# CityU-AIM-Group/SCAN

Hardware: AMD Instinct MI355X
Metric: train images/sec (whole node), VGG16 C2F 1024x2048 (higher is better)
Workload: dtype f32 (fp32 storage, fp32 multiply, fp32 accumulate -- the reference's arithmetic; the convolutions run it on the bf16 matrix cores as bf16x6: every fp32 operand cut into 3 bf16 pieces = all 24 significand bits, 6 bf16 MFMAs per product)

## Files before the change

include/scan_hip.h:

```cpp
#ifndef SCAN_HIP_H
#define SCAN_HIP_H

#include <stdint.h>

#ifdef __cplusplus
extern "C" {
#endif

#define SCAN_MAX_LEVELS 5

typedef struct {
  int32_t n_levels;
  int32_t n_images;
  int32_t h[SCAN_MAX_LEVELS];
  int32_t w[SCAN_MAX_LEVELS];
  int64_t row_off[SCAN_MAX_LEVELS + 1];
} scan_pyramid_t;

const char* scan_last_error(void);
int scan_abi_version(void);

#define SCAN_TUNE_UNKNOWN (-2147483647 - 1)
int scan_tune(const char* key, int value);
int scan_tune_get(const char* key);
// ... 47 lines not shown
int scan_cka_bce_forward_ordered(const float* logits, const float* act, int64_t M, int32_t Cf, float target, float* out,
                                 float* ws, void* stream);
int scan_cka_bce_forward_loss_ordered(const float* logits, const float* act, int64_t M, int32_t Cf, float target,
                                      float* out, float* ws, void* stream);
int64_t scan_softmax_focal_ordered_ws_floats(int64_t M);
int scan_softmax_focal_forward_ordered(const float* logits, const int64_t* labels, int64_t M, int32_t K, float gamma,
                                       float* loss_sum, float* ws, void* stream);

int scan_scale(const float* x, float alpha, float* y, int64_t n, void* stream);
int scan_copy_cols(const float* src, int32_t ld_src, float* dst, int32_t ld_dst, int64_t M, int32_t ncols, int32_t ztail,
                   void* stream);
int scan_paradigm_update(float* P, const float* pb, int32_t K, int32_t C, int32_t T, int32_t it, void* stream);

int32_t scan_dynconv_max_classes(void);
int scan_dynconv_softmax_forward(const float* feat, const float* kernels, int64_t M, int32_t C, int32_t K,
                                 float* logits, float* probs, void* stream);
int64_t scan_dynconv_ws_floats(int64_t M, int32_t C, int32_t K);
int scan_dynconv_softmax_backward(const float* feat, const float* kernels, const float* probs,
                                  const float* d_logits_in, const float* d_probs, int64_t M, int32_t C,
                                  int32_t K, float* d_feat, float* d_kernels, float* ws, void* stream);

int scan_softmax_focal_forward(const float* logits, const int64_t* labels, int64_t M, int32_t K, float gamma,
                               float* loss_sum, void* stream);
int scan_softmax_focal_backward(const float* logits, const int64_t* labels, int64_t M, int32_t K, float gamma,
                                float d_scale, float* d_logits, void* stream);

#define SCAN_NMS_PANEL 8192
#define SCAN_NMS_MAX 262144
int64_t scan_nms_ws_bytes(int64_t n);
int scan_nms(const float* dets, const float* scores, const float* labels, int64_t n, float thr, int32_t rule_ge,
             int64_t* keep_out, int32_t* num_keep_out, void* workspace, void* stream);

int scan_conv2d_forward(const float* x, const scan_pyramid_t* xd, int32_t Cin_s, const float* w, const float* bias,
                        float* y, const scan_pyramid_t* yd, int32_t Cout, int32_t Cout_s, int32_t ksize,
                        int32_t stride, int32_t relu, void* stream);
int scan_conv2d_dgrad(const float* dy, const scan_pyramid_t* yd, int32_t Cout_s, const float* wt, float* dx,
                      const scan_pyramid_t* xd, int32_t Cin, int32_t Cin_s, int32_t ksize, int32_t stride,
                      const float* mask, void* stream);
int64_t scan_conv2d_wgrad_ws_floats(const scan_pyramid_t* yd, int32_t Cin_s, int32_t Cout, int32_t ksize);
int scan_conv2d_wgrad(const float* x, const scan_pyramid_t* xd, int32_t Cin_s, const float* dy,
                      const scan_pyramid_t* yd, int32_t Cout, int32_t Cout_s, int32_t ksize, int32_t stride,
                      float* dw, int32_t accumulate, float* ws, void* stream);
int scan_weight_split(const float* w, int32_t O, int32_t T, int32_t Cs, int32_t mode, void* wh, void* wl,
                      int32_t Csw, void* stream);
int scan_conv3x3_bf16x3(const float* x, const scan_pyramid_t* d, int32_t Cs, const void* wh, const void* wl,
                        int32_t Csw, const float* bias, const float* mask, float* y, int32_t Nout, int32_t Ns,
                        int32_t relu, void* stream);
int scan_conv1x1_bf16x3(const float* x, const scan_pyramid_t* xd, int32_t Cs, const void* wh, const void* wl,
                        int32_t Csw, const float* bias, const float* mask, float* y, const scan_pyramid_t* yd,
                        int32_t Nout, int32_t Ns, int32_t relu, int32_t map, void* stream);
int64_t scan_conv1x1_wgrad_bf16x3_ws_floats(const scan_pyramid_t* yd, int32_t Cs, int32_t Cout);
int scan_conv1x1_wgrad_bf16x3(const float* x, const scan_pyramid_t* xd, int32_t Cs, const float* dy,
                              const scan_pyramid_t* yd, int32_t Cout, int32_t Cout_s, int32_t stride, float* dw,
                              float* db, int32_t accumulate, float* ws, void* stream);
int scan_conv_smallcin_bf16x3(const float* x, int32_t N, int32_t H, int32_t W, const float* w, const float* bias,
                              float* y, int32_t Cout, int32_t Cout_s, int32_t ksize, int32_t stride, int32_t relu,
                              void* stream);
int scan_conv3x3_gn_bf16x3(const float* x, const scan_pyramid_t* d, int32_t Cs, const void* wh, const void* wl,
                           int32_t Csw, const float* bias, float* y, int32_t Nout, int32_t Ns, float* gn_ws,
                           void* stream);
int scan_conv3x3_gn_acc_bf16x3(const float* x, const scan_pyramid_t* d, int32_t Cs, const void* wh, const void* wl,
                               int32_t Csw, const float* bias, float* y, int32_t Nout, int32_t Ns, float* gn_ws,
                               void* stream);
int scan_groupnorm_stats_from_sums(const float* ws, const scan_pyramid_t* d, int32_t C, int32_t G, float eps,
                                   float* stats, void* stream);
int scan_conv3x3_pool2_bf16x3(const float* x, const scan_pyramid_t* d, int32_t Cs, const void* wh, const void* wl,
                              int32_t Csw, const float* bias, float* y, int32_t Nout, int32_t Ns, int32_t relu,
                              void* stream);
int64_t scan_conv3x3_wgrad_bf16x3_ws_floats(const scan_pyramid_t* d, int32_t Cs, int32_t Cout);
int scan_conv3x3_wgrad_bf16x3(const float* x, const scan_pyramid_t* d, int32_t Cs, const float* dy, int32_t Cout,
                              int32_t Cout_s, float* dw, float* db, int32_t accumulate, float* ws, void* stream);
int scan_weight_split3(const float* w, int32_t O, int32_t T, int32_t Cs, int32_t mode, void* wh, void* wm, void* wl,
                       int32_t Csw, void* stream);
int scan_conv3x3_bf16x6(const float* x, const scan_pyramid_t* d, int32_t Cs, const void* wh, const void* wm,
                        const void* wl, int32_t Csw, const float* bias, const float* mask, float* y, int32_t Nout,
                        int32_t Ns, int32_t relu, void* stream);
int scan_conv1x1_bf16x6(const float* x, const scan_pyramid_t* xd, int32_t Cs, const void* wh, const void* wm,
                        const void* wl, int32_t Csw, const float* bias, const float* mask, float* y,
                        const scan_pyramid_t* yd, int32_t Nout, int32_t Ns, int32_t relu, int32_t map, void* stream);
int scan_conv3x3_gn_bf16x6(const float* x, const scan_pyramid_t* d, int32_t Cs, const void* wh, const void* wm,
                           const void* wl, int32_t Csw, const float* bias, float* y, int32_t Nout, int32_t Ns,
                           float* gn_ws, int32_t clear, void* stream);
int scan_conv3x3_pool2_bf16x6(const float* x, const scan_pyramid_t* d, int32_t Cs, const void* wh, const void* wm,
                              const void* wl, int32_t Csw, const float* bias, float* y, int32_t Nout, int32_t Ns,
                              int32_t relu, void* stream);
int scan_conv_smallcin_bf16x6(const float* x, int32_t N, int32_t H, int32_t W, const float* w, const float* bias,
                              float* y, int32_t Cout, int32_t Cout_s, int32_t ksize, int32_t stride, int32_t relu,
                              void* stream);
int64_t scan_conv3x3_wgrad_bf16x6_ws_floats(const scan_pyramid_t* d, int32_t Cs, int32_t Cout);
int scan_conv3x3_wgrad_bf16x6(const float* x, const scan_pyramid_t* d, int32_t Cs, const float* dy, int32_t Cout,
                              int32_t Cout_s, float* dw, float* db, int32_t accumulate, float* ws, void* stream);
int64_t scan_conv1x1_wgrad_bf16x6_ws_floats(const scan_pyramid_t* yd, int32_t Cs, int32_t Cout);
int scan_conv1x1_wgrad_bf16x6(const float* x, const scan_pyramid_t* xd, int32_t Cs, const float* dy,
                              const scan_pyramid_t* yd, int32_t Cout, int32_t Cout_s, int32_t stride, float* dw,
                              float* db, int32_t accumulate, float* ws, void* stream);
int scan_conv3x3_bf16x6_instance(const scan_pyramid_t* d, int32_t Nout);
int scan_conv3x3_wino_bf16x6(const float* x, const scan_pyramid_t* d, int32_t Cs, const void* wh, const void* wm,
                             const void* wl, int32_t Csw, const float* bias, const float* mask, float* y, int32_t Nout,
                             int32_t Ns, int32_t relu, float* gn_ws, int32_t clear, void* stream);
int scan_conv3x3_bf16x6_wino(int32_t Nout, int32_t Csw);
#define SCAN_CONV_SUMS 1
#define SCAN_CONV_POOL 2
#define SCAN_CONV_DIRECT3X3 0
#define SCAN_CONV_WINO3X3 1
#define SCAN_CONV_1X1 2
typedef struct {
  int32_t pieces;
  int32_t taps;
  int32_t dgrad;
  int32_t O, Cs_w;
  int32_t split_mode;
  int32_t plane_rows;
  int32_t plane_taps;
  int32_t csw;
  int32_t nout;
  int32_t rem;
  int32_t family;
  int32_t instance;
  int32_t flags;
} scan_conv_plan_t;
int scan_conv_plan(int32_t pieces, int32_t taps, int32_t dgrad, int32_t O, int32_t Cs_w, int32_t Cs_src,
                   const scan_pyramid_t* od, int32_t flags, scan_conv_plan_t* plan);
int scan_conv_weight_split(const scan_conv_plan_t* plan, const float* w, void* p0, void* p1, void* p2, void* stream);
int scan_conv_run(const scan_conv_plan_t* plan, const float* x, const scan_pyramid_t* xd, int32_t Cs, const void* p0,
                  const void* p1, const void* p2, const float* bias, const float* mask, float* y,
                  const scan_pyramid_t* yd, int32_t Ns, int32_t relu, int32_t map, float* gn_ws, int32_t clear,
                  void* stream);
#define SCAN_WGRAD_SPLIT3X3 1
#define SCAN_WGRAD_SPLIT1X1 2
#define SCAN_WGRAD_GENERIC 3
#define SCAN_WGRAD_FP32 0
#define SCAN_WGRAD_V4 1
#define SCAN_WGRAD_V6_64X32 2
#define SCAN_WGRAD_V6_32X64 3
#define SCAN_WGRAD_V6_32X64_WINO 4
typedef struct {
  int32_t family;
  int32_t pieces;
  int32_t ksize;
  int32_t stride;
  int32_t Cs, Cout;
  int32_t variant;
  int32_t wk;
  int32_t n_tiles;
  int32_t c_tiles;
  int32_t splits;
  int32_t cps;
  int32_t slab_taps;
  int32_t fused_db;
  int64_t chunks;
  int64_t slab_floats;
  int64_t bias_off;
  int64_t colsum_off;
  int64_t ws_floats;
} scan_conv_wgrad_plan_t;
int scan_conv_wgrad_plan(int32_t pieces, int32_t ksize, int32_t stride, int32_t Cs, int32_t Cout, const scan_pyramid_t* xd,
                         const scan_pyramid_t* yd, scan_conv_wgrad_plan_t* plan);
int scan_conv_wgrad_run(const scan_conv_wgrad_plan_t* plan, const float* x, const scan_pyramid_t* xd, int32_t Cs,
                        const float* dy, const scan_pyramid_t* yd, int32_t Cout, int32_t Cout_s, float* dw, float* db,
                        int32_t accumulate, float* ws, void* stream);
int scan_weight_transpose(const float* w, int32_t Cout, int32_t T, int32_t Cin_s, float* wt, int32_t Cout_s,
                          void* stream);
int64_t scan_colsum_ws_floats(int64_t M, int32_t C);
int scan_colsum(const float* dy, int64_t M, int32_t C, int32_t ld, float* db, int32_t accumulate, float* ws,
                void* stream);
int scan_relu_backward(const float* dy, const float* y, float* out, int64_t n, void* stream);

int scan_groupnorm_stats(const float* x, const scan_pyramid_t* d, int32_t C, int32_t G, float eps, float* stats,
                         float* ws, void* stream);
int scan_groupnorm_relu_forward(const float* x, const scan_pyramid_t* d, int32_t C, int32_t G, const float* stats,
                                const float* gamma, const float* beta, int32_t relu, float* y, void* stream);
int scan_groupnorm_relu_forward_from_sums(const float* x, const scan_pyramid_t* d, int32_t C, int32_t G,
                                          const float* sums, float eps, const float* gamma, const float* beta,
                                          int32_t relu, float* y, float* stats, void* stream);
int64_t scan_groupnorm_ws_floats(const scan_pyramid_t* d, int32_t C, int32_t G);
int scan_groupnorm_relu_backward(const float* x, const float* beta, const float* dy, const scan_pyramid_t* d, int32_t C,
                                 int32_t G, const float* stats, const float* gamma, int32_t relu, float* dx,
                                 float* dgamma, float* dbeta, int32_t accumulate, float* ws, void* stream);
int scan_groupnorm_relu_forward_ld(const float* x, const scan_pyramid_t* d, int32_t C, int32_t G, const float* stats,
                                   const float* gamma, const float* beta, int32_t relu, float* y, int32_t ldy,
                                   void* stream);
int scan_groupnorm_relu_forward_from_sums_ld(const float* x, const scan_pyramid_t* d, int32_t C, int32_t G,
                                             const float* sums, float eps, const float* gamma, const float* beta,
                                             int32_t relu, float* y, int32_t ldy, float* stats, void* stream);
int scan_groupnorm_relu_backward_ld(const float* x, const float* beta, const float* dy, int32_t lddy,
                                    const scan_pyramid_t* d, int32_t C, int32_t G, const float* stats, const float* gamma,
                                    int32_t relu, float* dx, float* dgamma, float* dbeta, int32_t accumulate, float* ws,
                                    void* stream);
int64_t scan_groupnorm_ordered_ws_floats(const scan_pyramid_t* d, int32_t C, int32_t G);
int scan_groupnorm_stats_ordered(const float* x, const scan_pyramid_t* d, int32_t C, int32_t G, float eps, float* stats,
                                 float* ws, void* stream);
int scan_groupnorm_relu_backward_ordered(const float* x, const float* beta, const float* dy, const scan_pyramid_t* d,
                                         int32_t C, int32_t G, const float* stats, const float* gamma, int32_t relu,
                                         float* dx, float* dgamma, float* dbeta, int32_t accumulate, float* ws,
                                         void* stream);
int scan_groupnorm_relu_backward_ld_ordered(const float* x, const float* beta, const float* dy, int32_t lddy,
                                            const scan_pyramid_t* d, int32_t C, int32_t G, const float* stats,
                                            const float* gamma, int32_t relu, float* dx, float* dgamma, float* dbeta,
                                            int32_t accumulate, float* ws, void* stream);
#define SCAN_GN_SUMS 1
#define SCAN_GN_SEPARATE_FINAL 2
#define SCAN_GN_FROM_X 0
#define SCAN_GN_FROM_SUMS 1
#define SCAN_GN_FROM_SUMS_FINAL 2
typedef struct {
  int32_t C, G;
  int32_t n_levels;
  int32_t n_images;
  int32_t blocks;
  int32_t ordered;
  int32_t source;
  int32_t stats_floats;
  int32_t fwd_ws_doubles;
  int32_t bwd_ws_doubles;
} scan_groupnorm_plan_t;
int scan_groupnorm_plan(const scan_pyramid_t* d, int32_t C, int32_t G, int32_t flags, scan_groupnorm_plan_t* plan);
int scan_groupnorm_run_forward(const scan_groupnorm_plan_t* plan, const float* x, const scan_pyramid_t* d, const float* sums,
                               float eps, const float* gamma, const float* beta, int32_t relu, float* y, int32_t ldy,
                               float* stats, float* ws, void* stream);
int scan_groupnorm_run_backward(const scan_groupnorm_plan_t* plan, const float* x, const float* beta, const float* dy,
                                int32_t lddy, const scan_pyramid_t* d, const float* stats, const float* gamma, int32_t relu,
                                float* dx, float* dgamma, float* dbeta, int32_t accumulate, float* ws, int32_t ws_cleared,
                                void* stream);

int scan_fcos_assign(const scan_pyramid_t* d, const int32_t* strides, const float* soi, const float* boxes,
                     const int64_t* glabels, const int32_t* ng, int32_t G, int64_t* labels, int32_t* labels_i32,
                     float* reg, int32_t* level_pos, void* stream);
int scan_fcos_compact(const scan_pyramid_t* d, const int64_t* labels, int32_t* pos_list, int32_t* neg_list, void* stream);
int64_t scan_fcos_nodes_count(const scan_pyramid_t* d, const int32_t* level_pos);
int scan_fcos_nodes(const scan_pyramid_t* d, const int32_t* level_pos, const int64_t* labels, const float* reg,
                    const int32_t* pos_list, const int32_t* neg_list, int64_t* node_index, int64_t* node_labels,
                    int64_t* pos_inds, float* reg_pos, float* ctr_pos, void* stream);

int64_t scan_atss_assign_ws_bytes(const scan_pyramid_t* d, int32_t G, int32_t topk);
int scan_atss_assign(const scan_pyramid_t* d, const int32_t* strides, const float* anchor_sizes, const float* boxes,
                     const int64_t* glabels, const int32_t* ng, int32_t G, int32_t topk, int64_t* labels,
                     int32_t* labels_i32, int32_t* matched, int32_t* level_pos, void* ws, void* stream);
int scan_atss_targets(const scan_pyramid_t* d, const int32_t* strides, const float* anchor_sizes, const int32_t* level_pos,
                      const float* boxes, int32_t G, const int32_t* matched, const int32_t* pos_list, int64_t* pos_inds,
                      float* reg_pos, float* ctr_pos, void* stream);
int scan_atss_giou_forward(const scan_pyramid_t* d, const int32_t* strides, const float* anchor_sizes, const float* pred,
                           const float* target, const int64_t* rows, const float* weight, int64_t P, float* out2,
                           void* stream);
int64_t scan_atss_giou_ordered_ws_floats(int64_t P);
int scan_atss_giou_forward_ordered(const scan_pyramid_t* d, const int32_t* strides, const float* anchor_sizes,
                                   const float* pred, const float* target, const int64_t* rows, const float* weight,
                                   int64_t P, float* out2, float* ws, void* stream);
int scan_atss_giou_backward(const scan_pyramid_t* d, const int32_t* strides, const float* anchor_sizes, const float* pred,
                            const float* target, const int64_t* rows, const float* weight, int64_t P,
                            const float* g_num_dev, float* d_pred, void* stream);

int scan_upsample2x_add(const float* lat, const float* coarse, int32_t N, int32_t h, int32_t w, int32_t C, float* y,
                        void* stream);
int scan_downsample2x_sum(const float* g, int32_t N, int32_t h, int32_t w, int32_t C, float* d, void* stream);

int scan_maxpool2x2_forward(const float* x, int32_t N, int32_t H, int32_t W, int32_t C, float* y, void* stream);
int scan_maxpool2x2_backward(const float* x, const float* y, const float* dy, int32_t N, int32_t H, int32_t W,
                             int32_t C, float* dx, int32_t relu_mask, void* stream);

int scan_maxpool3x3s2_forward(const float* x, int32_t N, int32_t H, int32_t W, int32_t C, float* y, void* stream);
int scan_add_relu(const float* a, const float* b, float* y, int64_t n, void* stream);

#define SCAN_DBSCAN_MAX 1200000
int64_t scan_dbscan_ws_bytes(int64_t n);
int scan_dbscan_prepare(const float* pts, int64_t n, int32_t D, float eps, int32_t min_samples, void* ws,
                        int32_t* info, void* stream);
int scan_dbscan_neighbor_counts(int64_t n, const void* ws, int32_t* counts, void* stream);
int scan_dbscan_bfs_step(int64_t n, void* ws, int32_t parity, int32_t* changed, void* stream);
int scan_dbscan_finish(int64_t n, void* ws, uint8_t* in_cluster0, void* stream);

int scan_sgd_momentum(float* p, const float* g, float* buf, int64_t n, float lr, float wd, float momentum,
                      int32_t first_step, void* stream);

#define SCAN_SGD_MAX_SEGMENTS 32
typedef struct {
  float* p;
  const float* g;
  float* buf;
  int64_t n;
  float lr;
  float wd;
  int32_t first_step;
  int32_t reserved;
} scan_sgd_segment_t;
int scan_sgd_momentum_multi(const scan_sgd_segment_t* segs, int32_t n_segs, float momentum, void* stream);

#define SCAN_SPLIT_JOB_WORDS 11
int64_t scan_weight_split_job_blocks(int32_t O, int32_t T, int32_t Cs, int32_t mode, int32_t Csw);
int scan_weight_split_batched(const int64_t* jobs, int32_t n_jobs, int32_t job_words, int64_t total_blocks, void* stream);

#define SCAN_CKA_MAX_CLASSES 16
typedef struct {
  const float* w0;
  const float* b0;
  const float* w2;
  const float* b2;
} scan_cka_branch_t;
int scan_cka_stack_weights(const scan_cka_branch_t* branches, int32_t Cf, int32_t C, int32_t H, int64_t s1o, int64_t s1c,
                           int64_t s1k, int64_t s2c, int64_t s2k, int32_t Cs1, int32_t Cs2, float* w1, float* b1,
                           float* w2, float* b2, void* stream);
int scan_cka_unstack_grads(const scan_cka_branch_t* grads, int32_t Cf, int32_t C, int32_t H, int64_t s1o, int64_t s1c,
                           int64_t s1k, int64_t s2c, int64_t s2k, int32_t Cs1, int32_t Cs2, const float* dw1,
                           const float* db1, const float* dw2, const float* db2, int32_t accumulate, void* stream);

int64_t scan_gconv3x3_to1_ws_floats(const scan_pyramid_t* d, int32_t G, int32_t Cg);
int scan_gconv3x3_to1_forward(const float* x, const scan_pyramid_t* d, int32_t G, int32_t Cg, const float* w,
                              const float* bias, float* y, int32_t Ns, float* ws, void* stream);
int scan_gconv3x3_to1_dgrad(const float* dy, int32_t Ns, const scan_pyramid_t* d, int32_t G, int32_t Cg, const float* w,
                            const float* mask, float* dx, void* stream);
int scan_gconv3x3_to1_wgrad(const float* x, const float* dy, int32_t Ns, const scan_pyramid_t* d, int32_t G, int32_t Cg,
                            float* dw, int32_t accumulate, float* ws, void* stream);
int scan_gconv3x3_to1_backward(const float* x, const float* dy, int32_t Ns, const scan_pyramid_t* d, int32_t G, int32_t Cg,
                               const float* w, int32_t relu_mask, float* dx, float* dw, int32_t accumulate, float* ws,
                               void* stream);
int32_t scan_gconv3x3_to1_max_groups(void);
int scan_gconv3x3_to1_any_forward(const float* x, const scan_pyramid_t* d, int32_t G, int32_t Cg, const float* w,
                                  const float* bias, float* y, int32_t Ns, float* ws, void* stream);
int scan_gconv3x3_to1_any_dgrad(const float* dy, int32_t Ns, const scan_pyramid_t* d, int32_t G, int32_t Cg, const float* w,
                                const float* mask, float* dx, void* stream);
int scan_gconv3x3_to1_any_wgrad(const float* x, const float* dy, int32_t Ns, const scan_pyramid_t* d, int32_t G, int32_t Cg,
                                float* dw, int32_t accumulate, float* ws, void* stream);
int scan_gconv3x3_to1_any_backward(const float* x, const float* dy, int32_t Ns, const scan_pyramid_t* d, int32_t G, int32_t Cg,
                                   const float* w, int32_t relu_mask, float* dx, float* dw, int32_t accumulate, float* ws,
                                   void* stream);
int scan_gconv3x3_to1_forward_bits(const float* x, const scan_pyramid_t* d, int32_t G, int32_t Cg, const float* w,
                                   const float* bias, float* y, int32_t Ns, float* ws, uint32_t* relu_bits, void* stream);
int scan_gconv3x3_to1_backward_bits(const float* x, const float* dy, int32_t Ns, const scan_pyramid_t* d, int32_t G,
                                    int32_t Cg, const float* w, const uint32_t* relu_bits, float* dx, float* dw,
                                    int32_t accumulate, float* ws, void* stream);

int scan_resize_bilinear_u8(const uint8_t* src, int32_t H, int32_t W, uint8_t* tmp, uint8_t* dst, int32_t OH, int32_t OW,
                            const int32_t* xbounds, const int32_t* xcoef, int32_t kx, const int32_t* ybounds,
                            const int32_t* ycoef, int32_t ky, void* stream);

int scan_normalize_image_u8(const uint8_t* src, int32_t H, int32_t W, int32_t flip, int32_t to_bgr255,
                            const float* mean3, const float* std3, float* dst, int32_t Hp, int32_t Wp, int32_t layout,
                            void* stream);

int scan_take_images_backward(const float* g, const scan_pyramid_t* d, int32_t i0, int32_t i1, int32_t C, float* out,
                              void* stream);

int scan_cond_rnn_forward(const float* x, int32_t K, int32_t T, const float* const* weights, float* h0, float* h1,
                          float* kernels, void* stream);
int64_t scan_cond_rnn_ws_floats(void);
int scan_cond_rnn_backward(const float* x, int32_t K, int32_t T, const float* const* weights, const float* h0,
                           const float* h1, const float* dkernels, float* const* grads, float* ws, void* stream);

#define SCAN_PACK_MAX_LEVELS 8
typedef struct {
  const float* data;
  int32_t h, w;
  int64_t sn, sc, sy, sx;
} scan_level_t;
int scan_pyramid_pack(const scan_level_t* levels, int32_t n_levels, int32_t n_images, int32_t C, float* rows, int32_t Cs,
                      void* stream);
int scan_pyramid_unpack(const float* rows, int32_t Cs, const scan_level_t* levels, int32_t n_levels, int32_t n_images,
                        int32_t C, void* stream);

int scan_deform_sample_forward(const float* x, const scan_pyramid_t* d, int32_t C, int32_t Cs, const float* off, int32_t ld_off,
                               const float* mask, int32_t ld_mask, float* cols, void* stream);
int scan_deform_sample_backward(const float* x, const scan_pyramid_t* d, int32_t C, int32_t Cs, const float* dcols, const float* off,
                                int32_t ld_off, const float* mask, int32_t ld_mask, float* doff, int32_t ld_doff, float* dmask,
                                int32_t ld_dmask, int32_t* keys, float* wgts, void* stream);
int scan_deform_dx_gather(const float* dcols, const int64_t* perm, const int64_t* seg_start, const float* wgts, int64_t M, int32_t C,
                          int32_t Cs, float* dx, void* stream);

int scan_center_aware_map(const float* cls, int32_t Cs, int32_t C, const float* ctr, int64_t ctr_stride, float weight, int64_t M,
                          float* atten, void* stream);
int scan_row_scale_levels(const float* x, int32_t ldx, const float* a, const float* s, const scan_pyramid_t* d, int32_t C, float* y,
                          int32_t ldy, void* stream);
int scan_row_scale_levels_ptrs(const float* const* x_levels, int32_t ldx, const float* a, const float* s, const scan_pyramid_t* d,
                               int32_t C, float* y, int32_t ldy, void* stream);

#ifdef __cplusplus
}
#endif
#endif
```

scan_amd/_lib.py:

```python
import ctypes
import os

_HERE = os.path.dirname(os.path.abspath(__file__))
LIB_PATH = os.environ.get("SCAN_HIP_LIB") or os.path.join(_HERE, "libscan_hip.so")

MAX_LEVELS = 5
TUNE_UNKNOWN = -2 ** 31
NMS_PANEL = 8192
NMS_MAX = 262144

c_i32, c_i64, c_f32, c_vp = ctypes.c_int32, ctypes.c_int64, ctypes.c_float, ctypes.c_void_p


class PyramidDesc(ctypes.Structure):
    _fields_ = [("n_levels", c_i32), ("n_images", c_i32), ("h", c_i32 * MAX_LEVELS), ("w", c_i32 * MAX_LEVELS),
                ("row_off", c_i64 * (MAX_LEVELS + 1))]


_PD = ctypes.POINTER(PyramidDesc)


class SgdSegment(ctypes.Structure):
    _fields_ = [("p", c_vp), ("g", c_vp), ("buf", c_vp), ("n", c_i64), ("lr", c_f32), ("wd", c_f32),
                ("first_step", c_i32), ("reserved", c_i32)]


class CkaBranch(ctypes.Structure):
    _fields_ = [("w0", c_vp), ("b0", c_vp), ("w2", c_vp), ("b2", c_vp)]


class LevelDesc(ctypes.Structure):
    _fields_ = [("data", c_vp), ("h", c_i32), ("w", c_i32), ("sn", c_i64), ("sc", c_i64), ("sy", c_i64), ("sx", c_i64)]


class ConvPlan(ctypes.Structure):
    _fields_ = [(n, c_i32) for n in ("pieces", "taps", "dgrad", "O", "Cs_w", "split_mode", "plane_rows", "plane_taps", "csw",
                                     "nout", "rem", "family", "instance", "flags")]


CONV_SUMS, CONV_POOL = 1, 2
_CP = ctypes.POINTER(ConvPlan)


class WgradPlan(ctypes.Structure):
    _fields_ = [(n, c_i32) for n in ("family", "pieces", "ksize", "stride", "Cs", "Cout", "variant", "wk", "n_tiles", "c_tiles",
                                     "splits", "cps", "slab_taps", "fused_db")] + \
               [(n, c_i64) for n in ("chunks", "slab_floats", "bias_off", "colsum_off", "ws_floats")]


WGRAD_SPLIT3X3, WGRAD_SPLIT1X1, WGRAD_GENERIC = 1, 2, 3
WGRAD_FP32, WGRAD_V4, WGRAD_V6_64X32, WGRAD_V6_32X64, WGRAD_V6_32X64_WINO = range(5)
_WP = ctypes.POINTER(WgradPlan)



class GroupNormPlan(ctypes.Structure):
    _fields_ = [(n, c_i32) for n in ("C", "G", "n_levels", "n_images", "blocks", "ordered", "source", "stats_floats",
                                     "fwd_ws_doubles", "bwd_ws_doubles")]


GN_SUMS, GN_SEPARATE_FINAL = 1, 2
GN_FROM_X, GN_FROM_SUMS, GN_FROM_SUMS_FINAL = range(3)
_GP = ctypes.POINTER(GroupNormPlan)

PACK_MAX_LEVELS = 8
SGD_MAX_SEGMENTS = 32
CKA_MAX_CLASSES = 16
SPLIT_JOB_WORDS = 11

SIGNATURES = {
    "scan_last_error": (ctypes.c_char_p, []),
    "scan_abi_version": (ctypes.c_int, []),
    "scan_comm_standin": (ctypes.c_int, [ctypes.c_void_p, ctypes.c_int64, ctypes.c_double, ctypes.c_int32, ctypes.c_double,
                                         ctypes.c_void_p]),
    "scan_tune": (ctypes.c_int, [ctypes.c_char_p, ctypes.c_int]),
    "scan_take_images_backward": (ctypes.c_int, [c_vp, _PD, c_i32, c_i32, c_i32, c_vp, c_vp]),
    "scan_cond_rnn_forward": (ctypes.c_int, [c_vp, c_i32, c_i32, c_vp, c_vp, c_vp, c_vp, c_vp]),
    "scan_cond_rnn_ws_floats": (ctypes.c_int64, []),
    "scan_cond_rnn_backward": (ctypes.c_int, [c_vp, c_i32, c_i32, c_vp, c_vp, c_vp, c_vp, c_vp, c_vp, c_vp]),
    "scan_tune_get": (ctypes.c_int, [ctypes.c_char_p]),
    "scan_tune_default": (ctypes.c_int, [ctypes.c_char_p]),
    "scan_tune_key": (ctypes.c_char_p, [ctypes.c_int]),
    "scan_mfma_sustained_bf16": (ctypes.c_int, [ctypes.c_double, c_i32, ctypes.POINTER(ctypes.c_double), c_vp]),
    "scan_conv3x3_bf16x3_instance": (ctypes.c_int, [_PD, c_i32]),
    "scan_conv1x1_bf16x6_instance": (ctypes.c_int, [_PD, c_i32, c_i32]),
    "scan_conv3x3_bf16x6_instance": (ctypes.c_int, [_PD, c_i32]),
    "scan_conv3x3_bf16x6_wino": (ctypes.c_int, [c_i32, c_i32]),
    "scan_conv3x3_wino_bf16x6": (ctypes.c_int, [c_vp, _PD, c_i32, c_vp, c_vp, c_vp, c_i32, c_vp, c_vp, c_vp, c_i32, c_i32, c_i32,
                                                c_vp, c_i32, c_vp]),
    "scan_conv_plan": (ctypes.c_int, [c_i32, c_i32, c_i32, c_i32, c_i32, c_i32, _PD, c_i32, _CP]),
    "scan_conv_weight_split": (ctypes.c_int, [_CP, c_vp, c_vp, c_vp, c_vp, c_vp]),
    "scan_conv_run": (ctypes.c_int, [_CP, c_vp, _PD, c_i32, c_vp, c_vp, c_vp, c_vp, c_vp, c_vp, _PD, c_i32, c_i32, c_i32, c_vp,
                                     c_i32, c_vp]),
    "scan_conv_wgrad_plan": (ctypes.c_int, [c_i32, c_i32, c_i32, c_i32, c_i32, _PD, _PD, _WP]),
    "scan_conv_wgrad_run": (ctypes.c_int, [_WP, c_vp, _PD, c_i32, c_vp, _PD, c_i32, c_i32, c_vp, c_vp, c_i32, c_vp, c_vp]),
    "scan_sigmoid_focal_loss_forward": (ctypes.c_int, [c_vp, c_vp, c_i64, c_i32, c_f32, c_f32, c_vp, c_vp, c_vp]),
    "scan_sigmoid_focal_loss_backward": (ctypes.c_int, [c_vp, c_vp, c_vp, c_f32, c_i64, c_i32, c_f32, c_f32, c_vp, c_vp]),
    "scan_iou_loss_forward": (ctypes.c_int, [c_vp, c_vp, c_vp, c_i64, c_vp, c_vp]),
    "scan_iou_loss_backward": (ctypes.c_int, [c_vp, c_vp, c_vp, c_i64, c_vp, c_vp, c_vp]),
    "scan_bce_logits_forward": (ctypes.c_int, [c_vp, c_vp, c_f32, c_vp, c_i64, c_i64, c_vp, c_vp]),
    "scan_bce_logits_backward": (ctypes.c_int, [c_vp, c_vp, c_f32, c_vp, c_i64, c_i64, c_vp, c_vp, c_vp]),
    "scan_cka_bce_forward": (ctypes.c_int, [c_vp, c_vp, c_i64, c_i32, c_f32, c_vp, c_vp]),
    "scan_cka_bce_backward": (ctypes.c_int, [c_vp, c_vp, c_i64, c_i32, c_f32, c_vp, c_vp, c_vp]),
    "scan_cka_bce_forward_loss": (ctypes.c_int, [c_vp, c_vp, c_i64, c_i32, c_f32, c_vp, c_vp]),
    "scan_cka_bce_backward_loss": (ctypes.c_int, [c_vp, c_vp, c_i64, c_i32, c_f32, c_vp, c_vp, c_vp, c_vp]),
    "scan_scale": (ctypes.c_int, [c_vp, c_f32, c_vp, c_i64, c_vp]),
    "scan_copy_cols": (ctypes.c_int, [c_vp, c_i32, c_vp, c_i32, c_i64, c_i32, c_i32, c_vp]),
    "scan_paradigm_update": (ctypes.c_int, [c_vp, c_vp, c_i32, c_i32, c_i32, c_i32, c_vp]),
    "scan_dynconv_softmax_forward": (ctypes.c_int, [c_vp, c_vp, c_i64, c_i32, c_i32, c_vp, c_vp, c_vp]),
    "scan_dynconv_ws_floats": (c_i64, [c_i64, c_i32, c_i32]),
    "scan_dynconv_max_classes": (c_i32, []),
    "scan_dynconv_softmax_backward": (ctypes.c_int, [c_vp, c_vp, c_vp, c_vp, c_vp, c_i64, c_i32, c_i32, c_vp, c_vp, c_vp, c_vp]),
    "scan_softmax_focal_forward": (ctypes.c_int, [c_vp, c_vp, c_i64, c_i32, c_f32, c_vp, c_vp]),
    "scan_softmax_focal_backward": (ctypes.c_int, [c_vp, c_vp, c_i64, c_i32, c_f32, c_f32, c_vp, c_vp]),
    "scan_nms_ws_bytes": (c_i64, [c_i64]),
    "scan_nms": (ctypes.c_int, [c_vp, c_vp, c_vp, c_i64, c_f32, c_i32, c_vp, c_vp, c_vp, c_vp]),
    "scan_conv2d_forward": (ctypes.c_int, [c_vp, _PD, c_i32, c_vp, c_vp, c_vp, _PD, c_i32, c_i32, c_i32, c_i32, c_i32, c_vp]),
    "scan_conv2d_dgrad": (ctypes.c_int, [c_vp, _PD, c_i32, c_vp, c_vp, _PD, c_i32, c_i32, c_i32, c_i32, c_vp, c_vp]),
    "scan_conv2d_wgrad_ws_floats": (c_i64, [_PD, c_i32, c_i32, c_i32]),
    "scan_conv2d_wgrad": (ctypes.c_int, [c_vp, _PD, c_i32, c_vp, _PD, c_i32, c_i32, c_i32, c_i32, c_vp, c_i32, c_vp, c_vp]),
    "scan_weight_split": (ctypes.c_int, [c_vp, c_i32, c_i32, c_i32, c_i32, c_vp, c_vp, c_i32, c_vp]),
    "scan_conv3x3_bf16x3": (ctypes.c_int, [c_vp, _PD, c_i32, c_vp, c_vp, c_i32, c_vp, c_vp, c_vp, c_i32, c_i32, c_i32, c_vp]),
    "scan_conv3x3_wgrad_bf16x3_ws_floats": (c_i64, [_PD, c_i32, c_i32]),
    "scan_dbscan_ws_bytes": (c_i64, [c_i64]),
    "scan_conv1x1_wgrad_bf16x3_ws_floats": (c_i64, [_PD, c_i32, c_i32]),
    "scan_conv3x3_wgrad_bf16x3": (ctypes.c_int, [c_vp, _PD, c_i32, c_vp, c_i32, c_i32, c_vp, c_vp, c_i32, c_vp, c_vp]),
    "scan_weight_transpose": (ctypes.c_int, [c_vp, c_i32, c_i32, c_i32, c_vp, c_i32, c_vp]),
    "scan_colsum_ws_floats": (c_i64, [c_i64, c_i32]),
    "scan_colsum": (ctypes.c_int, [c_vp, c_i64, c_i32, c_i32, c_vp, c_i32, c_vp, c_vp]),
    "scan_relu_backward": (ctypes.c_int, [c_vp, c_vp, c_vp, c_i64, c_vp]),
    "scan_groupnorm_stats": (ctypes.c_int, [c_vp, _PD, c_i32, c_i32, c_f32, c_vp, c_vp, c_vp]),
    "scan_groupnorm_relu_forward": (ctypes.c_int, [c_vp, _PD, c_i32, c_i32, c_vp, c_vp, c_vp, c_i32, c_vp, c_vp]),
    "scan_groupnorm_relu_forward_from_sums": (ctypes.c_int, [c_vp, _PD, c_i32, c_i32, c_vp, c_f32, c_vp, c_vp, c_i32, c_vp, c_vp, c_vp]),
    "scan_groupnorm_ws_floats": (c_i64, [_PD, c_i32, c_i32]),
    "scan_fcos_assign": (ctypes.c_int, [_PD, c_vp, c_vp, c_vp, c_vp, c_vp, c_i32, c_vp, c_vp, c_vp, c_vp, c_vp]),
    "scan_fcos_compact": (ctypes.c_int, [_PD, c_vp, c_vp, c_vp, c_vp]),
    "scan_fcos_nodes_count": (c_i64, [_PD, c_vp]),
    "scan_fcos_nodes": (ctypes.c_int, [_PD, c_vp, c_vp, c_vp, c_vp, c_vp, c_vp, c_vp, c_vp, c_vp, c_vp, c_vp]),
    "scan_atss_assign_ws_bytes": (c_i64, [_PD, c_i32, c_i32]),
    "scan_atss_assign": (ctypes.c_int, [_PD, c_vp, c_vp, c_vp, c_vp, c_vp, c_i32, c_i32, c_vp, c_vp, c_vp, c_vp, c_vp, c_vp]),
    "scan_atss_targets": (ctypes.c_int, [_PD, c_vp, c_vp, c_vp, c_vp, c_i32, c_vp, c_vp, c_vp, c_vp, c_vp, c_vp]),
    "scan_atss_giou_forward": (ctypes.c_int, [_PD, c_vp, c_vp, c_vp, c_vp, c_vp, c_vp, c_i64, c_vp, c_vp]),
    "scan_atss_giou_ordered_ws_floats": (c_i64, [c_i64]),
    "scan_atss_giou_forward_ordered": (ctypes.c_int, [_PD, c_vp, c_vp, c_vp, c_vp, c_vp, c_vp, c_i64, c_vp, c_vp, c_vp]),
    "scan_atss_giou_backward": (ctypes.c_int, [_PD, c_vp, c_vp, c_vp, c_vp, c_vp, c_vp, c_i64, c_vp, c_vp, c_vp]),
    "scan_groupnorm_relu_forward_ld": (ctypes.c_int, [c_vp, _PD, c_i32, c_i32, c_vp, c_vp, c_vp, c_i32, c_vp, c_i32, c_vp]),
    "scan_groupnorm_relu_forward_from_sums_ld": (ctypes.c_int, [c_vp, _PD, c_i32, c_i32, c_vp, c_f32, c_vp, c_vp, c_i32, c_vp,
                                                                c_i32, c_vp, c_vp]),
    "scan_groupnorm_relu_backward_ld": (ctypes.c_int, [c_vp, c_vp, c_vp, c_i32, _PD, c_i32, c_i32, c_vp, c_vp, c_i32, c_vp,
                                                       c_vp, c_vp, c_i32, c_vp, c_vp]),
    "scan_groupnorm_relu_backward": (ctypes.c_int, [c_vp, c_vp, c_vp, _PD, c_i32, c_i32, c_vp, c_vp, c_i32, c_vp, c_vp, c_vp, c_i32, c_vp, c_vp]),
    "scan_maxpool2x2_forward": (ctypes.c_int, [c_vp, c_i32, c_i32, c_i32, c_i32, c_vp, c_vp]),
    "scan_maxpool2x2_backward": (ctypes.c_int, [c_vp, c_vp, c_vp, c_i32, c_i32, c_i32, c_i32, c_vp, c_i32, c_vp]),
    "scan_conv3x3_gn_bf16x3": (ctypes.c_int, [c_vp, _PD, c_i32, c_vp, c_vp, c_i32, c_vp, c_vp, c_i32, c_i32, c_vp, c_vp]),
    "scan_conv3x3_gn_acc_bf16x3": (ctypes.c_int, [c_vp, _PD, c_i32, c_vp, c_vp, c_i32, c_vp, c_vp, c_i32, c_i32, c_vp, c_vp]),
    "scan_groupnorm_stats_from_sums": (ctypes.c_int, [c_vp, _PD, c_i32, c_i32, c_f32, c_vp, c_vp]),
    "scan_conv3x3_pool2_bf16x3": (ctypes.c_int, [c_vp, _PD, c_i32, c_vp, c_vp, c_i32, c_vp, c_vp, c_i32, c_i32, c_i32, c_vp]),
    "scan_conv1x1_bf16x3": (ctypes.c_int, [c_vp, _PD, c_i32, c_vp, c_vp, c_i32, c_vp, c_vp, c_vp, _PD, c_i32, c_i32, c_i32,
                                           c_i32, c_vp]),
    "scan_conv1x1_wgrad_bf16x3": (ctypes.c_int, [c_vp, _PD, c_i32, c_vp, _PD, c_i32, c_i32, c_i32, c_vp, c_vp, c_i32, c_vp,
                                                 c_vp]),
    "scan_conv_smallcin_bf16x3": (ctypes.c_int, [c_vp, c_i32, c_i32, c_i32, c_vp, c_vp, c_vp, c_i32, c_i32, c_i32, c_i32,
                                                 c_i32, c_vp]),
    "scan_weight_split3": (ctypes.c_int, [c_vp, c_i32, c_i32, c_i32, c_i32, c_vp, c_vp, c_vp, c_i32, c_vp]),
    "scan_conv3x3_bf16x6": (ctypes.c_int, [c_vp, _PD, c_i32, c_vp, c_vp, c_vp, c_i32, c_vp, c_vp, c_vp, c_i32, c_i32, c_i32, c_vp]),
    "scan_conv1x1_bf16x6": (ctypes.c_int, [c_vp, _PD, c_i32, c_vp, c_vp, c_vp, c_i32, c_vp, c_vp, c_vp, _PD, c_i32, c_i32, c_i32,
                                           c_i32, c_vp]),
    "scan_conv3x3_gn_bf16x6": (ctypes.c_int, [c_vp, _PD, c_i32, c_vp, c_vp, c_vp, c_i32, c_vp, c_vp, c_i32, c_i32, c_vp, c_i32,
                                              c_vp]),
    "scan_conv3x3_pool2_bf16x6": (ctypes.c_int, [c_vp, _PD, c_i32, c_vp, c_vp, c_vp, c_i32, c_vp, c_vp, c_i32, c_i32, c_i32,
                                                 c_vp]),
    "scan_conv3x3_wgrad_bf16x6_ws_floats": (c_i64, [_PD, c_i32, c_i32]),
    "scan_conv3x3_wgrad_bf16x6": (ctypes.c_int, [c_vp, _PD, c_i32, c_vp, c_i32, c_i32, c_vp, c_vp, c_i32, c_vp, c_vp]),
    "scan_conv1x1_wgrad_bf16x6_ws_floats": (c_i64, [_PD, c_i32, c_i32]),
    "scan_conv1x1_wgrad_bf16x6": (ctypes.c_int, [c_vp, _PD, c_i32, c_vp, _PD, c_i32, c_i32, c_i32, c_vp, c_vp, c_i32, c_vp,
                                                 c_vp]),
    "scan_conv_smallcin_bf16x6": (ctypes.c_int, [c_vp, c_i32, c_i32, c_i32, c_vp, c_vp, c_vp, c_i32, c_i32, c_i32, c_i32,
                                                 c_i32, c_vp]),
    "scan_maxpool3x3s2_forward": (ctypes.c_int, [c_vp, c_i32, c_i32, c_i32, c_i32, c_vp, c_vp]),
    "scan_upsample2x_add": (ctypes.c_int, [c_vp, c_vp, c_i32, c_i32, c_i32, c_i32, c_vp, c_vp]),
    "scan_downsample2x_sum": (ctypes.c_int, [c_vp, c_i32, c_i32, c_i32, c_i32, c_vp, c_vp]),
    "scan_add_relu": (ctypes.c_int, [c_vp, c_vp, c_vp, c_i64, c_vp]),
    "scan_dbscan_prepare": (ctypes.c_int, [c_vp, c_i64, c_i32, c_f32, c_i32, c_vp, c_vp, c_vp]),
    "scan_dbscan_neighbor_counts": (ctypes.c_int, [c_i64, c_vp, c_vp, c_vp]),
    "scan_dbscan_bfs_step": (ctypes.c_int, [c_i64, c_vp, c_i32, c_vp, c_vp]),
    "scan_dbscan_finish": (ctypes.c_int, [c_i64, c_vp, c_vp, c_vp]),
    "scan_sgd_momentum": (ctypes.c_int, [c_vp, c_vp, c_vp, c_i64, c_f32, c_f32, c_f32, c_i32, c_vp]),
    "scan_sgd_momentum_multi": (ctypes.c_int, [ctypes.POINTER(SgdSegment), c_i32, c_f32, c_vp]),
    "scan_weight_split_job_blocks": (c_i64, [c_i32, c_i32, c_i32, c_i32, c_i32]),
    "scan_weight_split_batched": (ctypes.c_int, [c_vp, c_i32, c_i32, c_i64, c_vp]),
    "scan_cka_stack_weights": (ctypes.c_int, [ctypes.POINTER(CkaBranch), c_i32, c_i32, c_i32, c_i64, c_i64, c_i64, c_i64,
                                              c_i64, c_i32, c_i32, c_vp, c_vp, c_vp, c_vp, c_vp]),
    "scan_cka_unstack_grads": (ctypes.c_int, [ctypes.POINTER(CkaBranch), c_i32, c_i32, c_i32, c_i64, c_i64, c_i64, c_i64,
                                              c_i64, c_i32, c_i32, c_vp, c_vp, c_vp, c_vp, c_i32, c_vp]),
    "scan_gconv3x3_to1_ws_floats": (c_i64, [_PD, c_i32, c_i32]),
    "scan_gconv3x3_to1_max_groups": (c_i32, []),
    "scan_gconv3x3_to1_any_forward": (ctypes.c_int, [c_vp, _PD, c_i32, c_i32, c_vp, c_vp, c_vp, c_i32, c_vp, c_vp]),
    "scan_gconv3x3_to1_any_dgrad": (ctypes.c_int, [c_vp, c_i32, _PD, c_i32, c_i32, c_vp, c_vp, c_vp, c_vp]),
    "scan_gconv3x3_to1_any_wgrad": (ctypes.c_int, [c_vp, c_vp, c_i32, _PD, c_i32, c_i32, c_vp, c_i32, c_vp, c_vp]),
    "scan_gconv3x3_to1_any_backward": (ctypes.c_int, [c_vp, c_vp, c_i32, _PD, c_i32, c_i32, c_vp, c_i32, c_vp, c_vp, c_i32,
                                                      c_vp, c_vp]),
    "scan_gconv3x3_to1_forward": (ctypes.c_int, [c_vp, _PD, c_i32, c_i32, c_vp, c_vp, c_vp, c_i32, c_vp, c_vp]),
    "scan_gconv3x3_to1_dgrad": (ctypes.c_int, [c_vp, c_i32, _PD, c_i32, c_i32, c_vp, c_vp, c_vp, c_vp]),
    "scan_gconv3x3_to1_wgrad": (ctypes.c_int, [c_vp, c_vp, c_i32, _PD, c_i32, c_i32, c_vp, c_i32, c_vp, c_vp]),
    "scan_gconv3x3_to1_backward": (ctypes.c_int, [c_vp, c_vp, c_i32, _PD, c_i32, c_i32, c_vp, c_i32, c_vp, c_vp, c_i32, c_vp,
                                                  c_vp]),
    "scan_gconv3x3_to1_forward_bits": (ctypes.c_int, [c_vp, _PD, c_i32, c_i32, c_vp, c_vp, c_vp, c_i32, c_vp, c_vp, c_vp]),
    "scan_gconv3x3_to1_backward_bits": (ctypes.c_int, [c_vp, c_vp, c_i32, _PD, c_i32, c_i32, c_vp, c_vp, c_vp, c_vp, c_i32,
                                                       c_vp, c_vp]),
    "scan_resize_bilinear_u8": (ctypes.c_int, [c_vp, c_i32, c_i32, c_vp, c_vp, c_i32, c_i32, c_vp, c_vp, c_i32, c_vp, c_vp,
                                               c_i32, c_vp]),
    "scan_sigmoid_focal_loss_ordered_ws_floats": (c_i64, [c_i64, c_i32]),
    "scan_sigmoid_focal_loss_forward_ordered": (ctypes.c_int, [c_vp, c_vp, c_i64, c_i32, c_f32, c_f32, c_vp, c_vp, c_vp, c_vp]),
    "scan_iou_loss_ordered_ws_floats": (c_i64, [c_i64]),
    "scan_iou_loss_forward_ordered": (ctypes.c_int, [c_vp, c_vp, c_vp, c_i64, c_vp, c_vp, c_vp]),
    "scan_bce_logits_ordered_ws_floats": (c_i64, [c_i64]),
    "scan_bce_logits_forward_ordered": (ctypes.c_int, [c_vp, c_vp, c_f32, c_vp, c_i64, c_i64, c_vp, c_vp, c_vp]),
    "scan_cka_bce_ordered_ws_floats": (c_i64, [c_i64, c_i32]),
    "scan_cka_bce_forward_ordered": (ctypes.c_int, [c_vp, c_vp, c_i64, c_i32, c_f32, c_vp, c_vp, c_vp]),
    "scan_cka_bce_forward_loss_ordered": (ctypes.c_int, [c_vp, c_vp, c_i64, c_i32, c_f32, c_vp, c_vp, c_vp]),
    "scan_softmax_focal_ordered_ws_floats": (c_i64, [c_i64]),
    "scan_softmax_focal_forward_ordered": (ctypes.c_int, [c_vp, c_vp, c_i64, c_i32, c_f32, c_vp, c_vp, c_vp]),
    "scan_groupnorm_ordered_ws_floats": (c_i64, [_PD, c_i32, c_i32]),
    "scan_groupnorm_stats_ordered": (ctypes.c_int, [c_vp, _PD, c_i32, c_i32, c_f32, c_vp, c_vp, c_vp]),
    "scan_groupnorm_relu_backward_ordered": (ctypes.c_int, [c_vp, c_vp, c_vp, _PD, c_i32, c_i32, c_vp, c_vp, c_i32, c_vp, c_vp, c_vp,
                                                            c_i32, c_vp, c_vp]),
    "scan_groupnorm_relu_backward_ld_ordered": (ctypes.c_int, [c_vp, c_vp, c_vp, c_i32, _PD, c_i32, c_i32, c_vp, c_vp, c_i32, c_vp,
                                                               c_vp, c_vp, c_i32, c_vp, c_vp]),
    "scan_groupnorm_plan": (ctypes.c_int, [_PD, c_i32, c_i32, c_i32, _GP]),
    "scan_groupnorm_run_forward": (ctypes.c_int, [_GP, c_vp, _PD, c_vp, c_f32, c_vp, c_vp, c_i32, c_vp, c_i32, c_vp, c_vp, c_vp]),
    "scan_groupnorm_run_backward": (ctypes.c_int, [_GP, c_vp, c_vp, c_vp, c_i32, _PD, c_vp, c_vp, c_i32, c_vp, c_vp, c_vp, c_i32,
                                                   c_vp, c_i32, c_vp]),
    "scan_normalize_image_u8": (ctypes.c_int, [c_vp, c_i32, c_i32, c_i32, c_i32, ctypes.POINTER(c_f32),
                                               ctypes.POINTER(c_f32), c_vp, c_i32, c_i32, c_i32, c_vp]),
    "scan_pyramid_pack": (ctypes.c_int, [ctypes.POINTER(LevelDesc), c_i32, c_i32, c_i32, c_vp, c_i32, c_vp]),
    "scan_pyramid_unpack": (ctypes.c_int, [c_vp, c_i32, ctypes.POINTER(LevelDesc), c_i32, c_i32, c_i32, c_vp]),
    "scan_deform_sample_forward": (ctypes.c_int, [c_vp, _PD, c_i32, c_i32, c_vp, c_i32, c_vp, c_i32, c_vp, c_vp]),
    "scan_deform_sample_backward": (ctypes.c_int, [c_vp, _PD, c_i32, c_i32, c_vp, c_vp, c_i32, c_vp, c_i32, c_vp, c_i32, c_vp,
                                                   c_i32, c_vp, c_vp, c_vp]),
    "scan_deform_dx_gather": (ctypes.c_int, [c_vp, c_vp, c_vp, c_vp, c_i64, c_i32, c_i32, c_vp, c_vp]),
    "scan_center_aware_map": (ctypes.c_int, [c_vp, c_i32, c_i32, c_vp, c_i64, c_f32, c_i64, c_vp, c_vp]),
    "scan_row_scale_levels": (ctypes.c_int, [c_vp, c_i32, c_vp, ctypes.POINTER(c_f32), _PD, c_i32, c_vp, c_i32, c_vp]),
    "scan_row_scale_levels_ptrs": (ctypes.c_int, [ctypes.POINTER(c_vp), c_i32, c_vp, ctypes.POINTER(c_f32), _PD, c_i32, c_vp, c_i32,
                                                  c_vp]),
}

_lib = None


def lib():
    global _lib
    if _lib is None:
        if not os.path.exists(LIB_PATH):
            raise RuntimeError(
                "scan_amd: %s is missing -- build it with `python -c 'import __graft_entry__ as g; g.build()'` "
                "(hipcc --offload-arch=gfx950); there is no CPU fallback." % LIB_PATH)
        import torch
        L = ctypes.CDLL(LIB_PATH)
        for name, (res, args) in SIGNATURES.items():
            fn = getattr(L, name)
            fn.restype = res
            fn.argtypes = args
        for kv in filter(None, os.environ.get("SCAN_TUNE", "").split(",")):
            key, _, val = kv.partition("=")
            if L.scan_tune(key.strip().encode(), int(val)) == TUNE_UNKNOWN:
                raise RuntimeError("SCAN_TUNE: unknown key %r" % key)
        _lib = L
    return _lib


def tune_state():
    L, out, i = lib(), {}, 0
    while True:
        k = L.scan_tune_key(i)
        if k is None:
            return out
        out[k.decode()] = (L.scan_tune_get(k), L.scan_tune_default(k))
        i += 1


def lib_identity():
    import hashlib
    with open(LIB_PATH, "rb") as f:
        sha = hashlib.sha1(f.read()).hexdigest()
    product = os.path.realpath(LIB_PATH) == os.path.realpath(os.path.join(_HERE, "libscan_hip.so"))
    return {"lib": os.path.basename(LIB_PATH), "lib_sha1": sha, "product_library": product,
            "scan_tune_non_default": {k: v for k, (v, d) in tune_state().items() if v != d}}


def call(name, *args):
    rc = getattr(lib(), name)(*args)
    if rc != 0:
        raise RuntimeError("%s failed (%d): %s" % (name, rc, lib().scan_last_error().decode()))


def query(name, *args):
    return getattr(lib(), name)(*args)
```

scan_amd/csrc/batched.hip:

```cpp
#include "conv_split.h"

#define SPLIT_ELEMS_PER_BLOCK 2048
#define SPLIT_TILE 64

__device__ __forceinline__ void split8_store(const float (&v)[8], __bf16* __restrict__ w0, __bf16* __restrict__ w1,
                                             __bf16* __restrict__ w2, int64_t i) {
  bf16x8 q0, q1, q2;
#pragma unroll
  for (int k = 0; k < 8; ++k) {
    __bf16 q[3];
    split1_np<3>(v[k], q);
    q0[k] = q[0];
    q1[k] = q[1];
    q2[k] = q[2];
  }
  *reinterpret_cast<bf16x8*>(w0 + i) = q0;
  *reinterpret_cast<bf16x8*>(w1 + i) = q1;
  if (w2 != nullptr) *reinterpret_cast<bf16x8*>(w2 + i) = q2;
}

__global__ __launch_bounds__(256) void weight_split_batched_kernel(const int64_t* __restrict__ jobs, int n_jobs) {
  __shared__ float tile[SPLIT_TILE][SPLIT_TILE + 1];
  int j = 0;
  for (int i = 1; i < n_jobs; ++i)
    if ((int64_t)blockIdx.x >= jobs[(int64_t)i * SCAN_SPLIT_JOB_WORDS + 9]) j = i;
  const int64_t* job = jobs + (int64_t)j * SCAN_SPLIT_JOB_WORDS;
  const float* __restrict__ w = reinterpret_cast<const float*>(job[0]);
  __bf16* __restrict__ wh = reinterpret_cast<__bf16*>(job[1]);
  __bf16* __restrict__ wl = reinterpret_cast<__bf16*>(job[2]);
  __bf16* __restrict__ w2 = reinterpret_cast<__bf16*>(job[10]);
  const int O = (int)job[3], T = (int)job[4], Cs = (int)job[5], mode = (int)job[6], rows = (int)job[7],
            Csw = (int)job[8];
  const int64_t blk = (int64_t)blockIdx.x - job[9];
  const int tid = threadIdx.x;
  if (mode == 2) {
    const int64_t total = (int64_t)rows * 12 * Csw;
    const int64_t i = blk * SPLIT_ELEMS_PER_BLOCK + (int64_t)tid * 8;
    if (i >= total) return;
    const int col = (int)(i % Csw);
    const int64_t rt = i / Csw;
    const int tt = (int)(rt % 12), row = (int)(rt / 12);
    const int j = tt / 3, ky = tt - 3 * j;
    const float* src = w + ((int64_t)row * T + ky * 3) * Cs + col;
    float v[8];
#pragma unroll
    for (int k = 0; k < 8; ++k) {
      const bool in = col + k < Cs;
      v[k] = wino_g(j, in ? src[k] : 0.f, in ? src[Cs + k] : 0.f, in ? src[2 * Cs + k] : 0.f);
    }
    split8_store(v, wh, wl, w2, i);
    return;
  }
  if (mode == 0) {
    const int64_t total = (int64_t)rows * T * Csw;
    const int64_t i = blk * SPLIT_ELEMS_PER_BLOCK + (int64_t)tid * 8;
    if (i >= total) return;
    const int col = (int)(i % Csw);
    const int64_t rt = i / Csw;
    const float* src = w + rt * Cs + col;
    float v[8];
    if (col + 8 <= Cs && (Cs & 3) == 0) {
      const float4 a = *reinterpret_cast<const float4*>(src);
      const float4 b = *reinterpret_cast<const float4*>(src + 4);
      v[0] = a.x; v[1] = a.y; v[2] = a.z; v[3] = a.w;
      v[4] = b.x; v[5] = b.y; v[6] = b.z; v[7] = b.w;
    } else {
#pragma unroll
      for (int k = 0; k < 8; ++k) v[k] = (col + k < Cs) ? src[k] : 0.f;
    }
    split8_store(v, wh, wl, w2, i);
    return;
  }
  const int tiles_o = (Csw + SPLIT_TILE - 1) / SPLIT_TILE, tiles_c = (rows + SPLIT_TILE - 1) / SPLIT_TILE;
  const int to = (int)(blk % tiles_o);
  const int tc = (int)((blk / tiles_o) % tiles_c);
  const int tt = (int)(blk / ((int64_t)tiles_o * tiles_c));
  const int TO = mode == 3 ? 12 : T;
  const int o0 = to * SPLIT_TILE, c0 = tc * SPLIT_TILE;
  {
    const int cl = (tid & 15) * 4, ol = tid >> 4;
#pragma unroll
    for (int p = 0; p < SPLIT_TILE / 16; ++p) {
      const int o = o0 + ol + 16 * p, c = c0 + cl;
      float4 a = make_float4(0.f, 0.f, 0.f, 0.f);
      if (o < O && c < Cs) {
        auto read4 = [&](int t) {
          const float* src = w + ((int64_t)o * T + t) * Cs + c;
          float4 r = make_float4(0.f, 0.f, 0.f, 0.f);
          if (c + 4 <= Cs && (Cs & 3) == 0) {
            r = *reinterpret_cast<const float4*>(src);
          } else {
            r.x = src[0];
            if (c + 1 < Cs) r.y = src[1];
            if (c + 2 < Cs) r.z = src[2];
            if (c + 3 < Cs) r.w = src[3];
          }
          return r;
        };
        if (mode == 1) {
          a = read4(T - 1 - tt);
        } else {
          const int j = tt / 3, ky = tt - 3 * j;
          const float4 g0 = read4(8 - ky * 3), g1 = read4(7 - ky * 3), g2 = read4(6 - ky * 3);
          a = make_float4(wino_g(j, g0.x, g1.x, g2.x), wino_g(j, g0.y, g1.y, g2.y), wino_g(j, g0.z, g1.z, g2.z),
                          wino_g(j, g0.w, g1.w, g2.w));
        }
      }
      float* t = &tile[ol + 16 * p][cl];
      t[0] = a.x; t[1] = a.y; t[2] = a.z; t[3] = a.w;
    }
  }
  __syncthreads();
  {
    const int o8 = (tid & 7) * 8, cl = tid >> 3;
#pragma unroll
    for (int p = 0; p < SPLIT_TILE / 32; ++p) {
      const int c = c0 + cl + 32 * p, o = o0 + o8;
      if (c < rows && o < Csw) {
        float v[8];
#pragma unroll
        for (int k = 0; k < 8; ++k) v[k] = tile[o8 + k][cl + 32 * p];
        split8_store(v, wh, wl, w2, ((int64_t)c * TO + tt) * Csw + o);
      }
    }
  }
}

extern "C" int64_t scan_weight_split_job_blocks(int32_t O, int32_t T, int32_t Cs, int32_t mode, int32_t Csw) {
  const int64_t TO = mode >= 2 ? 12 : T;
  if (mode == 0 || mode == 2) return ((int64_t)O * TO * Csw + SPLIT_ELEMS_PER_BLOCK - 1) / SPLIT_ELEMS_PER_BLOCK;
  const int64_t tiles_o = (Csw + SPLIT_TILE - 1) / SPLIT_TILE, tiles_c = (Cs + SPLIT_TILE - 1) / SPLIT_TILE;
  return tiles_o * tiles_c * TO;
}

extern "C" int scan_weight_split_batched(const int64_t* jobs, int32_t n_jobs, int32_t job_words, int64_t total_blocks,
                                         void* stream) {
  SCAN_CHECK_ARG(job_words == SCAN_SPLIT_JOB_WORDS, "weight_split_batched: records of %d words, this library reads %d",
                 job_words, SCAN_SPLIT_JOB_WORDS);
  SCAN_CHECK_ARG(jobs && n_jobs > 0 && total_blocks > 0 && total_blocks < (1ll << 31),
                 "weight_split_batched: bad arguments (n_jobs=%d)", n_jobs);
  hipLaunchKernelGGL(weight_split_batched_kernel, dim3((unsigned)total_blocks), dim3(256), 0, as_stream(stream), jobs,
                     n_jobs);
  SCAN_LAUNCH_CHECK("weight_split_batched");
  return 0;
}

struct SgdSegs {
  scan_sgd_segment_t s[SCAN_SGD_MAX_SEGMENTS];
  int64_t first_block[SCAN_SGD_MAX_SEGMENTS + 1];
  int n;
};
#define SGD_ELEMS_PER_BLOCK 4096

__global__ __launch_bounds__(256) void sgd_multi_kernel(SgdSegs t, float momentum) {
  int j = 0;
#pragma unroll
  for (int i = 1; i < SCAN_SGD_MAX_SEGMENTS; ++i)
    if (i < t.n && (int64_t)blockIdx.x >= t.first_block[i]) j = i;
  const scan_sgd_segment_t sg = t.s[j];
  const int64_t base = ((int64_t)blockIdx.x - t.first_block[j]) * SGD_ELEMS_PER_BLOCK;
  float* __restrict__ p = sg.p;
  const float* __restrict__ g = sg.g;
  float* __restrict__ buf = sg.buf;
#pragma unroll 4
  for (int k = 0; k < SGD_ELEMS_PER_BLOCK / 256; ++k) {
    const int64_t i = base + k * 256 + threadIdx.x;
    if (i >= sg.n) break;
    const float w = p[i];
    const float gg = g[i] + sg.wd * w;
    const float b = sg.first_step ? gg : momentum * buf[i] + gg;
    buf[i] = b;
    p[i] = w - sg.lr * b;
  }
}

extern "C" int scan_sgd_momentum_multi(const scan_sgd_segment_t* segs, int32_t n_segs, float momentum, void* stream) {
  SCAN_CHECK_ARG(segs && n_segs > 0 && n_segs <= SCAN_SGD_MAX_SEGMENTS, "sgd_momentum_multi: n_segs=%d out of 1..%d", n_segs,
                 SCAN_SGD_MAX_SEGMENTS);
  SgdSegs t;
  t.n = 0;
  int64_t blocks = 0;
  for (int i = 0; i < n_segs; ++i) {
    SCAN_CHECK_ARG(segs[i].n >= 0, "sgd_momentum_multi: segment %d has n < 0", i);
    if (segs[i].n == 0) continue;
    SCAN_CHECK_ARG(segs[i].p && segs[i].g && segs[i].buf, "sgd_momentum_multi: null pointer in segment %d", i);
    t.s[t.n] = segs[i];
    t.first_block[t.n] = blocks;
    blocks += (segs[i].n + SGD_ELEMS_PER_BLOCK - 1) / SGD_ELEMS_PER_BLOCK;
    ++t.n;
  }
  if (t.n == 0) return 0;
  t.first_block[t.n] = blocks;
  SCAN_CHECK_ARG(blocks < (1ll << 31), "sgd_momentum_multi: too many elements");
  hipLaunchKernelGGL(sgd_multi_kernel, dim3((unsigned)blocks), dim3(256), 0, as_stream(stream), t, momentum);
  SCAN_LAUNCH_CHECK("sgd_momentum_multi");
  return 0;
}

struct CkaPtrs {
  scan_cka_branch_t b[SCAN_CKA_MAX_CLASSES];
};

__global__ __launch_bounds__(256) void cka_stack_kernel(CkaPtrs P, int Cf, int C, int H, int64_t s1o, int64_t s1c,
                                                        int64_t s1k, int64_t s2c, int64_t s2k, int Cs1, int Cs2,
                                                        float* __restrict__ w1, float* __restrict__ b1,
                                                        float* __restrict__ w2, float* __restrict__ b2) {
  const int64_t n1 = (int64_t)Cf * H * 9 * Cs1;
  const int64_t n2 = (int64_t)Cf * 9 * Cs2;
  const int64_t nb = (int64_t)Cf * H + Cf;
  for (int64_t i = (int64_t)blockIdx.x * blockDim.x + threadIdx.x; i < n1 + n2 + nb;
       i += (int64_t)gridDim.x * blockDim.x) {
    if (i < n1) {
      const int col = (int)(i % Cs1);
      const int64_t r = i / Cs1;
      const int k = (int)(r % 9);
      const int row = (int)(r / 9);
      const int c = row / H, o = row - c * H;
      float v = 0.f;
      if (col < C) v = P.b[c].w0[o * s1o + col * s1c + k * s1k];
      else if (col == C + c) v = P.b[c].w0[o * s1o + C * s1c + k * s1k];
      w1[i] = v;
    } else if (i < n1 + n2) {
      const int64_t q = i - n1;
      const int col = (int)(q % Cs2);
      const int64_t r = q / Cs2;
      const int k = (int)(r % 9);
      const int c = (int)(r / 9);
      float v = 0.f;
      if (col >= c * H && col < (c + 1) * H) v = P.b[c].w2[(col - c * H) * s2c + k * s2k];
      w2[q] = v;
    } else {
      const int q = (int)(i - n1 - n2);
      if (q < Cf * H) b1[q] = P.b[q / H].b0[q % H];
      else b2[q - Cf * H] = P.b[q - Cf * H].b2[0];
    }
  }
}

__global__ __launch_bounds__(256) void cka_unstack_kernel(CkaPtrs G, int Cf, int C, int H, int64_t s1o, int64_t s1c,
                                                          int64_t s1k, int64_t s2c, int64_t s2k, int Cs1, int Cs2,
                                                          const float* __restrict__ dw1, const float* __restrict__ db1,
                                                          const float* __restrict__ dw2, const float* __restrict__ db2,
                                                          int accumulate) {
  const int64_t n1 = (int64_t)Cf * H * 9 * (C + 1);
  const int64_t n2 = (int64_t)Cf * 9 * H;
  const int64_t nb = (int64_t)Cf * H + Cf;
  for (int64_t i = (int64_t)blockIdx.x * blockDim.x + threadIdx.x; i < n1 + n2 + nb;
       i += (int64_t)gridDim.x * blockDim.x) {
    if (i < n1) {
      const int col = (int)(i % (C + 1));
      const int64_t r = i / (C + 1);
      const int k = (int)(r % 9);
      const int row = (int)(r / 9);
      const int c = row / H, o = row - c * H;
      if (dw1 != nullptr) {
        const float v = dw1[((int64_t)row * 9 + k) * Cs1 + (col < C ? col : C + c)];
        float* dst = const_cast<float*>(G.b[c].w0) + o * s1o + col * s1c + k * s1k;
        *dst = accumulate ? *dst + v : v;
      }
    } else if (i < n1 + n2) {
      const int64_t q = i - n1;
      const int h = (int)(q % H);
      const int64_t r = q / H;
      const int k = (int)(r % 9);
      const int c = (int)(r / 9);
      if (dw2 != nullptr) {
        const float v = dw2[((int64_t)c * 9 + k) * Cs2 + c * H + h];
        float* dst = const_cast<float*>(G.b[c].w2) + h * s2c + k * s2k;
        *dst = accumulate ? *dst + v : v;
      }
    } else {
      const int q = (int)(i - n1 - n2);
      if (q < Cf * H) {
        if (db1 != nullptr) {
          float* dst = const_cast<float*>(G.b[q / H].b0) + q % H;
          *dst = accumulate ? *dst + db1[q] : db1[q];
        }
      } else if (db2 != nullptr) {
        float* dst = const_cast<float*>(G.b[q - Cf * H].b2);
        *dst = accumulate ? *dst + db2[q - Cf * H] : db2[q - Cf * H];
      }
    }
  }
}

static int cka_check(const scan_cka_branch_t* br, int Cf, int C, int H, int Cs1, int Cs2, const char* who) {
  SCAN_CHECK_ARG(br && Cf >= 1 && Cf <= SCAN_CKA_MAX_CLASSES, "%s: Cf=%d out of 1..%d", who, Cf, SCAN_CKA_MAX_CLASSES);
  SCAN_CHECK_ARG(C > 0 && H > 0 && Cs1 >= C + Cf && Cs2 >= Cf * H, "%s: C=%d H=%d Cs1=%d Cs2=%d", who, C, H, Cs1, Cs2);
  for (int c = 0; c < Cf; ++c)
    SCAN_CHECK_ARG(br[c].w0 && br[c].b0 && br[c].w2 && br[c].b2, "%s: null pointer in branch %d", who, c);
  return 0;
}

extern "C" int scan_cka_stack_weights(const scan_cka_branch_t* branches, int32_t Cf, int32_t C, int32_t H,
                                      int64_t s1o, int64_t s1c, int64_t s1k, int64_t s2c, int64_t s2k, int32_t Cs1,
                                      int32_t Cs2, float* w1, float* b1, float* w2, float* b2, void* stream) {
  if (cka_check(branches, Cf, C, H, Cs1, Cs2, "cka_stack_weights")) return -1;
  SCAN_CHECK_ARG(w1 && b1 && w2 && b2, "cka_stack_weights: null output");
  CkaPtrs P;
  for (int c = 0; c < Cf; ++c) P.b[c] = branches[c];
  const int64_t n = (int64_t)Cf * H * 9 * Cs1 + (int64_t)Cf * 9 * Cs2 + (int64_t)Cf * H + Cf;
  hipLaunchKernelGGL(cka_stack_kernel, dim3(grid_for(n, 256)), dim3(256), 0, as_stream(stream), P, Cf, C, H, s1o, s1c,
                     s1k, s2c, s2k, Cs1, Cs2, w1, b1, w2, b2);
  SCAN_LAUNCH_CHECK("cka_stack_weights");
  return 0;
}

extern "C" int scan_cka_unstack_grads(const scan_cka_branch_t* grads, int32_t Cf, int32_t C, int32_t H, int64_t s1o,
                                      int64_t s1c, int64_t s1k, int64_t s2c, int64_t s2k, int32_t Cs1, int32_t Cs2,
                                      const float* dw1, const float* db1, const float* dw2, const float* db2,
                                      int32_t accumulate, void* stream) {
  if (cka_check(grads, Cf, C, H, Cs1, Cs2, "cka_unstack_grads")) return -1;
  CkaPtrs G;
  for (int c = 0; c < Cf; ++c) G.b[c] = grads[c];
  const int64_t n = (int64_t)Cf * H * 9 * (C + 1) + (int64_t)Cf * 9 * H + (int64_t)Cf * H + Cf;
  hipLaunchKernelGGL(cka_unstack_kernel, dim3(grid_for(n, 256)), dim3(256), 0, as_stream(stream), G, Cf, C, H, s1o, s1c,
                     s1k, s2c, s2k, Cs1, Cs2, dw1, db1, dw2, db2, accumulate);
  SCAN_LAUNCH_CHECK("cka_unstack_grads");
  return 0;
}
```

scan_amd/csrc/gconv.hip:

```cpp
#include "common.h"

#define GC_G 128

template <int CTRL, int ROW_MASK>
__device__ __forceinline__ float dpp_add(float v) {
  const int r = __builtin_amdgcn_update_dpp(0, __builtin_bit_cast(int, v), CTRL, ROW_MASK, 0xF, false);
  return v + __builtin_bit_cast(float, r);
}
__device__ __forceinline__ float half_wave_sum_hi(float v) {
  v = dpp_add<0xB1, 0xF>(v);
  v = dpp_add<0x4E, 0xF>(v);
  v = dpp_add<0x141, 0xF>(v);
  v = dpp_add<0x140, 0xF>(v);
  v = dpp_add<0x142, 0xA>(v);
  return v;
}

__device__ __forceinline__ int64_t neighbour_row(const scan_pyramid_t& d, int64_t m, const RowCoord& rc, int oy, int ox) {
  const int y = rc.y + oy, x = rc.x + ox;
  if (y < 0 || y >= d.h[rc.lvl] || x < 0 || x >= d.w[rc.lvl]) return -1;
  return m + (int64_t)oy * d.w[rc.lvl] + ox;
}

#define GC_UNROLL 2
// ... 322 lines not shown
      for (int t = 0; t < 9; ++t) {
        float s = __fmaf_rn(h[u].x, wv[t].x, __fmaf_rn(h[u].y, wv[t].y, __fmaf_rn(h[u].z, wv[t].z, h[u].w * wv[t].w)));
        s = half_wave_sum_hi(s);
        if (l32 == 16 + t) mine = s;
      }
      if (q < M && l32 >= 16 && l32 < 25) T[(q * G + g) * 9 + (l32 - 16)] = mine;
    }
  }
}

template <bool DO_DX, bool DO_DW>
__global__ __launch_bounds__(256, 4) void gconv_bwd_generic_kernel(const float* __restrict__ x, const float* __restrict__ dy,
                                                                   int Ns, scan_pyramid_t d, int G, int GC,
                                                                   const float* __restrict__ w, int relu_mask,
                                                                   float* __restrict__ dx, float* __restrict__ slab) {
  const int64_t M = d.row_off[d.n_levels];
  const int hw = blockIdx.x * 8 + (threadIdx.x >> 5), l32 = threadIdx.x & 31;
  const int g = hw % G;
  const int64_t J = (int64_t)gridDim.x * 8 / G;
  const int64_t coff = (int64_t)g * GC_G + 4 * l32;
  float4 wv[9], acc[9];
#pragma unroll
  for (int t = 0; t < 9; ++t) {
    wv[t] = DO_DX ? *reinterpret_cast<const float4*>(w + ((int64_t)g * 9 + t) * GC + coff) : make_float4(0.f, 0.f, 0.f, 0.f);
    acc[t] = make_float4(0.f, 0.f, 0.f, 0.f);
  }
  const bool need_x = DO_DW || relu_mask;
  constexpr int UN = (DO_DX && DO_DW) ? 1 : GC_UNROLL;
  for (int64_t q0 = hw / G; q0 < M; q0 += UN * J) {
    float4 h[UN];
    float gy[UN][9];
#pragma unroll
    for (int u = 0; u < UN; ++u) {
      const int64_t q = q0 + u * J;
      h[u] = (q < M && need_x) ? *reinterpret_cast<const float4*>(x + q * GC + coff) : make_float4(0.f, 0.f, 0.f, 0.f);
      if (q < M) {
        const RowCoord rc = decode_row(d, q);
#pragma unroll
        for (int t = 0; t < 9; ++t) {
          const int64_t p = neighbour_row(d, q, rc, 1 - t / 3, 1 - t % 3);
          gy[u][t] = p >= 0 ? dy[p * Ns + g] : 0.f;
        }
      } else {
#pragma unroll
        for (int t = 0; t < 9; ++t) gy[u][t] = 0.f;
      }
    }
#pragma unroll
    for (int u = 0; u < UN; ++u) {
      const int64_t q = q0 + u * J;
      if (DO_DW) {
#pragma unroll
        for (int t = 0; t < 9; ++t) {
          acc[t].x = __fmaf_rn(gy[u][t], h[u].x, acc[t].x);
          acc[t].y = __fmaf_rn(gy[u][t], h[u].y, acc[t].y);
          acc[t].z = __fmaf_rn(gy[u][t], h[u].z, acc[t].z);
          acc[t].w = __fmaf_rn(gy[u][t], h[u].w, acc[t].w);
        }
      }
      if (DO_DX && q < M) {
        float4 o = make_float4(0.f, 0.f, 0.f, 0.f);
#pragma unroll
        for (int t = 0; t < 9; ++t) {
          o.x = __fmaf_rn(gy[u][t], wv[t].x, o.x);
          o.y = __fmaf_rn(gy[u][t], wv[t].y, o.y);
          o.z = __fmaf_rn(gy[u][t], wv[t].z, o.z);
          o.w = __fmaf_rn(gy[u][t], wv[t].w, o.w);
        }
        if (relu_mask) {
          o.x = h[u].x > 0.f ? o.x : 0.f;
          o.y = h[u].y > 0.f ? o.y : 0.f;
          o.z = h[u].z > 0.f ? o.z : 0.f;
          o.w = h[u].w > 0.f ? o.w : 0.f;
        }
        *reinterpret_cast<float4*>(dx + q * GC + coff) = o;
      }
    }
  }
  if (!DO_DW) return;
  float* out = slab + (int64_t)hw * 9 * GC_G + 4 * l32;
#pragma unroll
  for (int t = 0; t < 9; ++t) *reinterpret_cast<float4*>(out + t * GC_G) = acc[t];
}

__global__ __launch_bounds__(256) void gconv_wgrad_reduce_generic_kernel(const float* __restrict__ partial, int parts, int G,
                                                                         int GC, float* __restrict__ dw, int accumulate) {
  const int i = blockIdx.x * blockDim.x + threadIdx.x;
  if (i >= 9 * GC) return;
  const int gt = i / GC_G, c = i - gt * GC_G;
  float s = 0.f;
  for (int b = 0; b < parts; ++b) s += partial[(int64_t)b * 9 * GC + i];
  float* dst = dw + (int64_t)gt * GC + (gt / 9) * GC_G + c;
  *dst = accumulate ? *dst + s : s;
}

#define GC_MAX_BLOCKS 1024
#define GC_PARTS 32
#define GC_GMAX 31

static int gconv_check(const scan_pyramid_t* d, int G, int Cg, const char* who, bool any_g = false) {
  SCAN_CHECK_ARG(d && d->n_levels >= 1 && d->n_levels <= SCAN_MAX_LEVELS, "%s: bad pyramid", who);
  SCAN_CHECK_ARG(Cg == GC_G, "%s: only 128 channels per group are built (got %d)", who, Cg);
  if (any_g) {
    SCAN_CHECK_ARG(G >= 1 && G <= GC_GMAX, "%s: G=%d out of 1..%d", who, G, GC_GMAX);
    return 0;
  }
  SCAN_CHECK_ARG(G == 1 || G == 2 || G == 4 || G == 8, "%s: G=%d must be 1, 2, 4 or 8", who, G);
  return 0;
}

static bool gconv_generic(int G) { return !(G == 1 || G == 2 || G == 4 || G == 8); }

extern "C" int32_t scan_gconv3x3_to1_max_groups(void) { return GC_GMAX; }

static int gconv_generic_strides(int64_t M, int per, int max_j) {
  int64_t j = ((M + per - 1) / per + 7) / 8 * 8;
  if (j < 8) j = 8;
  if (j > max_j) j = max_j;
  return (int)j;
}

extern "C" int64_t scan_gconv3x3_to1_ws_floats(const scan_pyramid_t* d, int32_t G, int32_t Cg) {
  if (!d) return -1;
  const int64_t M = d->row_off[d->n_levels];
  const int64_t taps = M * G * 9;
  const int64_t slab = (int64_t)(GC_MAX_BLOCKS + GC_PARTS) * 9 * G * Cg;
  return taps > slab ? taps : slab;
}

int g_scan_gconv_mfma = 0;

static int gconv_wave_grid(int64_t M, int G) {
  int64_t tasks = ((M + 15) / 16) * G;
  int64_t blocks = (tasks + 3) / 4;
  if (blocks > 2048) blocks = 2048;
  if (blocks < 2) blocks = 2;
  return (int)((blocks + 1) / 2 * 2);
}

static int gconv_forward(const float* x, const scan_pyramid_t* d, int G, int Cg, const float* w, const float* bias, float* y,
                         int Ns, float* ws, uint32_t* relu_bits, hipStream_t st, bool any_g = false) {
  if (gconv_check(d, G, Cg, "gconv3x3_to1_forward", any_g)) return -1;
  SCAN_CHECK_ARG(x && w && y && ws && Ns >= G, "gconv3x3_to1_forward: bad arguments (Ns=%d)", Ns);
  const int64_t M = d->row_off[d->n_levels];
  if (M == 0) return 0;
  const int GC = G * Cg, slots = 256 / (GC / 4);
  if (gconv_generic(G)) {
    SCAN_CHECK_ARG(relu_bits == nullptr, "gconv3x3_to1_forward_bits: G=%d must be 1, 2, 4 or 8", G);
    const int J = gconv_generic_strides(M, GC_UNROLL_F, 2048);
    hipLaunchKernelGGL(gconv_taps_generic_kernel, dim3(J / 8 * G), dim3(256), 0, st, x, M, G, GC, w, ws);
    SCAN_LAUNCH_CHECK("gconv_taps_generic");
    hipLaunchKernelGGL(gconv_gather_kernel, dim3(grid_for(M * Ns, 256)), dim3(256), 0, st, ws, *d, G, bias, y, Ns);
    SCAN_LAUNCH_CHECK("gconv_gather");
    return 0;
  }
  if (g_scan_gconv_mfma || relu_bits != nullptr) {
    hipLaunchKernelGGL(gconv_taps_mfma_kernel, dim3(gconv_wave_grid(M, G)), dim3(256), 0, st, x, M, G, GC, w, ws, relu_bits);
  } else {
    hipLaunchKernelGGL(gconv_taps_kernel, dim3(grid_for((M + slots - 1) / slots, 1)), dim3(256), 0, st, x, M, G, GC, w, ws);
  }
  SCAN_LAUNCH_CHECK("gconv_taps");
  hipLaunchKernelGGL(gconv_gather_kernel, dim3(grid_for(M * Ns, 256)), dim3(256), 0, st, ws, *d, G, bias, y, Ns);
  SCAN_LAUNCH_CHECK("gconv_gather");
  return 0;
}

extern "C" int scan_gconv3x3_to1_forward(const float* x, const scan_pyramid_t* d, int32_t G, int32_t Cg, const float* w,
                                         const float* bias, float* y, int32_t Ns, float* ws, void* stream) {
  return gconv_forward(x, d, G, Cg, w, bias, y, Ns, ws, nullptr, as_stream(stream));
}

extern "C" int scan_gconv3x3_to1_forward_bits(const float* x, const scan_pyramid_t* d, int32_t G, int32_t Cg,
                                              const float* w, const float* bias, float* y, int32_t Ns, float* ws,
                                              uint32_t* relu_bits, void* stream) {
  SCAN_CHECK_ARG(relu_bits, "gconv3x3_to1_forward_bits: null bit mask");
  return gconv_forward(x, d, G, Cg, w, bias, y, Ns, ws, relu_bits, as_stream(stream));
}

static int gconv_backward(const float* x, const float* dy, int Ns, const scan_pyramid_t* d, int G, int Cg, const float* w,
                          int relu_mask, const uint32_t* relu_bits, float* dx, float* dw, int accumulate, float* ws,
                          hipStream_t st, const char* who, bool any_g = false) {
  if (gconv_check(d, G, Cg, who, any_g)) return -1;
  SCAN_CHECK_ARG(dy && Ns >= G && (dx || dw), "%s: bad arguments (Ns=%d)", who, Ns);
  SCAN_CHECK_ARG(!dx || w, "%s: the data gradient needs the weights", who);
  SCAN_CHECK_ARG(!dw || (x && ws), "%s: the weight gradient needs x and a workspace", who);
  SCAN_CHECK_ARG(!(dx && relu_mask && !relu_bits) || x, "%s: the ReLU mask needs x or its bit mask", who);
  const int64_t M = d->row_off[d->n_levels];
  if (M == 0) return 0;
  const int GC = G * Cg;
  if (gconv_generic(G)) {
    SCAN_CHECK_ARG(relu_bits == nullptr, "%s: G=%d must be 1, 2, 4 or 8", who, G);
    const int J = gconv_generic_strides(M, 16, GC_MAX_BLOCKS);
    const dim3 grid(J / 8 * G);
    if (dx && dw)
      hipLaunchKernelGGL((gconv_bwd_generic_kernel<true, true>), grid, dim3(256), 0, st, x, dy, Ns, *d, G, GC, w, relu_mask, dx, ws);
    else if (dx)
      hipLaunchKernelGGL((gconv_bwd_generic_kernel<true, false>), grid, dim3(256), 0, st, x, dy, Ns, *d, G, GC, w, relu_mask, dx,
                         ws);
    else
      hipLaunchKernelGGL((gconv_bwd_generic_kernel<false, true>), grid, dim3(256), 0, st, x, dy, Ns, *d, G, GC, w, 0, dx, ws);
    SCAN_LAUNCH_CHECK(who);
    if (dw) {
      const int n = 9 * GC, per = (J + GC_PARTS - 1) / GC_PARTS, parts = (J + per - 1) / per;
      float* partial = ws + (int64_t)GC_MAX_BLOCKS * n;
      hipLaunchKernelGGL(gconv_slab_partial_kernel, dim3((n + 255) / 256, parts), dim3(256), 0, st, ws, J, n, per, partial);
      SCAN_LAUNCH_CHECK("gconv_slab_partial");
      hipLaunchKernelGGL(gconv_wgrad_reduce_generic_kernel, dim3((n + 255) / 256), dim3(256), 0, st, partial, parts, G, GC, dw,
                         accumulate);
      SCAN_LAUNCH_CHECK("gconv_wgrad_reduce");
    }
    return 0;
  }
  int blocks = GC_MAX_BLOCKS;
  int64_t rpb = (M + blocks - 1) / blocks;
  if (rpb < 16) rpb = 16;
  blocks = (int)((M + rpb - 1) / rpb);
  const bool mfma = g_scan_gconv_mfma || relu_bits != nullptr;
  if (dx && mfma) {
    hipLaunchKernelGGL(gconv_dx_mfma_kernel, dim3(gconv_wave_grid(M, G)), dim3(256), 0, st, dy, Ns, *d, G, GC, w,
                       (relu_mask && !relu_bits) ? x : (const float*)nullptr, relu_bits, dx);
    SCAN_LAUNCH_CHECK(who);
    if (dw) hipLaunchKernelGGL((gconv_bwd_kernel<false, true>), dim3(blocks), dim3(256), 0, st, x, dy, Ns, *d, G, GC, w, 0,
                               dx, rpb, ws);
  } else if (dx && dw) {
    hipLaunchKernelGGL((gconv_bwd_kernel<true, true>), dim3(blocks), dim3(256), 0, st, x, dy, Ns, *d, G, GC, w, relu_mask, dx,
                       rpb, ws);
  } else if (dx) {
    hipLaunchKernelGGL((gconv_bwd_kernel<true, false>), dim3(blocks), dim3(256), 0, st, x, dy, Ns, *d, G, GC, w, relu_mask, dx,
                       rpb, ws);
  } else {
    hipLaunchKernelGGL((gconv_bwd_kernel<false, true>), dim3(blocks), dim3(256), 0, st, x, dy, Ns, *d, G, GC, w, 0, dx, rpb,
                       ws);
  }
  SCAN_LAUNCH_CHECK(who);
  if (dw) {
    const int n = 9 * GC, per = (blocks + GC_PARTS - 1) / GC_PARTS, parts = (blocks + per - 1) / per;
    float* partial = ws + (int64_t)GC_MAX_BLOCKS * n;
    hipLaunchKernelGGL(gconv_slab_partial_kernel, dim3((n + 255) / 256, parts), dim3(256), 0, st, ws, blocks, n, per,
                       partial);
    SCAN_LAUNCH_CHECK("gconv_slab_partial");
    hipLaunchKernelGGL(gconv_wgrad_reduce_kernel, dim3((n + 255) / 256), dim3(256), 0, st, partial, parts, G, GC, dw,
                       accumulate);
    SCAN_LAUNCH_CHECK("gconv_wgrad_reduce");
  }
  return 0;
}

extern "C" int scan_gconv3x3_to1_dgrad(const float* dy, int32_t Ns, const scan_pyramid_t* d, int32_t G, int32_t Cg,
                                       const float* w, const float* mask, float* dx, void* stream) {
  SCAN_CHECK_ARG(dx, "gconv3x3_to1_dgrad: null output");
  return gconv_backward(mask, dy, Ns, d, G, Cg, w, mask != nullptr, nullptr, dx, nullptr, 0, nullptr, as_stream(stream),
                        "gconv3x3_to1_dgrad");
}

extern "C" int scan_gconv3x3_to1_wgrad(const float* x, const float* dy, int32_t Ns, const scan_pyramid_t* d, int32_t G,
                                       int32_t Cg, float* dw, int32_t accumulate, float* ws, void* stream) {
  SCAN_CHECK_ARG(dw, "gconv3x3_to1_wgrad: null output");
  return gconv_backward(x, dy, Ns, d, G, Cg, nullptr, 0, nullptr, nullptr, dw, accumulate, ws, as_stream(stream),
                        "gconv3x3_to1_wgrad");
}

extern "C" int scan_gconv3x3_to1_backward(const float* x, const float* dy, int32_t Ns, const scan_pyramid_t* d, int32_t G,
                                          int32_t Cg, const float* w, int32_t relu_mask, float* dx, float* dw,
                                          int32_t accumulate, float* ws, void* stream) {
  SCAN_CHECK_ARG(x && dx && dw, "gconv3x3_to1_backward: null pointer");
  return gconv_backward(x, dy, Ns, d, G, Cg, w, relu_mask, nullptr, dx, dw, accumulate, ws, as_stream(stream),
                        "gconv3x3_to1_backward");
}

extern "C" int scan_gconv3x3_to1_backward_bits(const float* x, const float* dy, int32_t Ns, const scan_pyramid_t* d,
                                               int32_t G, int32_t Cg, const float* w, const uint32_t* relu_bits, float* dx,
                                               float* dw, int32_t accumulate, float* ws, void* stream) {
  SCAN_CHECK_ARG(x && dx && dw && relu_bits, "gconv3x3_to1_backward_bits: null pointer");
  return gconv_backward(x, dy, Ns, d, G, Cg, w, 1, relu_bits, dx, dw, accumulate, ws, as_stream(stream),
                        "gconv3x3_to1_backward_bits");
}

extern "C" int scan_gconv3x3_to1_any_forward(const float* x, const scan_pyramid_t* d, int32_t G, int32_t Cg, const float* w,
                                             const float* bias, float* y, int32_t Ns, float* ws, void* stream) {
  return gconv_forward(x, d, G, Cg, w, bias, y, Ns, ws, nullptr, as_stream(stream), true);
}

extern "C" int scan_gconv3x3_to1_any_dgrad(const float* dy, int32_t Ns, const scan_pyramid_t* d, int32_t G, int32_t Cg,
                                           const float* w, const float* mask, float* dx, void* stream) {
  SCAN_CHECK_ARG(dx, "gconv3x3_to1_any_dgrad: null output");
  return gconv_backward(mask, dy, Ns, d, G, Cg, w, mask != nullptr, nullptr, dx, nullptr, 0, nullptr, as_stream(stream),
                        "gconv3x3_to1_any_dgrad", true);
}

extern "C" int scan_gconv3x3_to1_any_wgrad(const float* x, const float* dy, int32_t Ns, const scan_pyramid_t* d, int32_t G,
                                           int32_t Cg, float* dw, int32_t accumulate, float* ws, void* stream) {
  SCAN_CHECK_ARG(dw, "gconv3x3_to1_any_wgrad: null output");
  return gconv_backward(x, dy, Ns, d, G, Cg, nullptr, 0, nullptr, nullptr, dw, accumulate, ws, as_stream(stream),
                        "gconv3x3_to1_any_wgrad", true);
}

extern "C" int scan_gconv3x3_to1_any_backward(const float* x, const float* dy, int32_t Ns, const scan_pyramid_t* d, int32_t G,
                                              int32_t Cg, const float* w, int32_t relu_mask, float* dx, float* dw,
                                              int32_t accumulate, float* ws, void* stream) {
  SCAN_CHECK_ARG(x && dx && dw, "gconv3x3_to1_any_backward: null pointer");
  return gconv_backward(x, dy, Ns, d, G, Cg, w, relu_mask, nullptr, dx, dw, accumulate, ws, as_stream(stream),
                        "gconv3x3_to1_any_backward", true);
}
```

scan_amd/modeling/discriminator.py:

```python
import torch
from torch import nn

from .. import ops
from ..layers import GradientReversal
from .backbone import conv_holder
from .fcos import make_tower, run_tower


def _check_epm_keywords(name, grl_applied_domain, patch_stride=None, center_aware_type=None):
    if grl_applied_domain != "both":
        raise ValueError("%s: grl_applied_domain %r is not built (MODEL.ADV.GRL_APPLIED_DOMAIN: only 'both')"
                         % (name, grl_applied_domain))
    if patch_stride is not None:
        raise ValueError("%s: patch_stride %r is not built (MODEL.ADV.PATCH_STRIDE: only None)" % (name, patch_stride))
    if center_aware_type is not None and center_aware_type not in ("ca_feature", "ca_loss"):
        raise ValueError("%s: center_aware_type %r is not built (MODEL.ADV.CENTER_AWARE_TYPE: 'ca_feature' or 'ca_loss')"
                         % (name, center_aware_type))


class FCOSDiscriminator(nn.Module):

    def __init__(self, num_convs=2, in_channels=256, grad_reverse_lambda=-1.0, grl_applied_domain="both", patch_stride=None):
        super().__init__()
        _check_epm_keywords(type(self).__name__, grl_applied_domain, patch_stride)
        if num_convs < 0 or in_channels != 256:
            raise ValueError("%s: num_convs %r >= 0 on 256 input channels is what is built (in_channels %r)"
                             % (type(self).__name__, num_convs, in_channels))
        self.num_convs = num_convs
        self.in_channels = in_channels
        self.dis_tower = make_tower(num_convs, in_channels)
        self.cls_logits = conv_holder(in_channels, 1, 3)
        for modules in (self.dis_tower, self.cls_logits):
            for m in modules.modules():
                if isinstance(m, nn.Conv2d):
                    nn.init.normal_(m.weight, std=0.01)
                    nn.init.constant_(m.bias, 0)
        self.grad_reverse = GradientReversal(grad_reverse_lambda)
        self.grl_applied_domain = grl_applied_domain

    def _logits(self, feature, shape):
        x = run_tower(self.dis_tower, feature, shape, self.num_convs)
        return ops.conv2d(x, self.cls_logits.weight, self.cls_logits.bias, shape, 3, 1)[:, 0]

    def forward(self, feature, target, domain="source", shape=None):
        assert target in (0, 1, 0.1, 0.9) and domain in ("source", "target")
        return ops.bce_with_logits_const_mean(self._logits(self.grad_reverse(feature), shape), target)

    def forward_pair(self, feature, shape, n_src, grl_applied=False):
        if not grl_applied:
            feature = self.grad_reverse(feature)
        (h, w) = shape.sizes[0]
        ls, lt = ops.split_rows2(self._logits(feature, shape), n_src * h * w)
        return ops.bce_with_logits_const_mean(ls, 1.0), ops.bce_with_logits_const_mean(lt, 0.0)


class FCOSDiscriminator_CA(FCOSDiscriminator):

    def __init__(self, num_convs=2, in_channels=256, grad_reverse_lambda=-1.0, center_aware_weight=0.0,
                 center_aware_type="ca_loss", grl_applied_domain="both"):
        _check_epm_keywords(type(self).__name__, grl_applied_domain, None, center_aware_type)
        super().__init__(num_convs, in_channels, grad_reverse_lambda, grl_applied_domain)
        self.center_aware_weight = center_aware_weight
        self.center_aware_type = center_aware_type

    def atten_map(self, score_map):
        cls = score_map["box_cls"]
        return ops.center_aware_map(cls, score_map["centerness"], cls.shape[1], self.center_aware_weight)

    def _input(self, feature, atten, shape):
        if self.center_aware_type == "ca_feature":
            return ops.center_aware_split_levels_grl(feature, atten, shape, [self.grad_reverse.lambda_])[0]
        return self.grad_reverse(feature)

    def _loss(self, logits, atten, target):
        return ops.bce_with_logits_const_mean(logits, target, atten if self.center_aware_type == "ca_loss" else None)

    def forward(self, feature, target, score_map=None, domain="source", shape=None):
        assert target in (0, 1, 0.1, 0.9) and domain in ("source", "target")
        atten = self.atten_map(score_map)
        return self._loss(self._logits(self._input(feature, atten, shape), shape), atten, target)

    def forward_pair(self, feature, atten, shape, n_src, grl_applied=False):
        if not grl_applied:
            feature = self._input(feature, atten, shape)
        (h, w) = shape.sizes[0]
        m = n_src * h * w
        ls, lt = ops.split_rows2(self._logits(feature, shape), m)
        return self._loss(ls, atten[:m], 1.0), self._loss(lt, atten[m:], 0.0)


class FCOSDiscriminator_con(nn.Module):
    def __init__(self, with_GA=False, fusion_cfg="concat", num_convs=4, in_channels=256, num_classes=9,
                 grad_reverse_lambda=0.02, grl_applied_domain="both", patch_stride=None, cfg=None):
        super().__init__()
        assert fusion_cfg == "concat" and grl_applied_domain == "both" and patch_stride is None and num_classes >= 2, \
            "only the configuration the SCAN yamls use is built"
        self.num_convs = num_convs
        self.in_channels = in_channels
        self.num_classes = num_classes - 1
        self.dis_tower = make_tower(num_convs, in_channels)
        for c in range(self.num_classes):
            self.add_module("classifier_cls_%d" % c, nn.Sequential(
                conv_holder(in_channels + 1, 128, 3), nn.ReLU(), conv_holder(128, 1, 3)))
        for m in self.modules():
            if isinstance(m, nn.Conv2d):
                nn.init.normal_(m.weight, std=0.01)
                nn.init.constant_(m.bias, 0)
        self.grad_reverse = GradientReversal(grad_reverse_lambda)

    def _stacked_weights_torch(self):
        Cf, C = self.num_classes, self.in_channels
        blocks = [getattr(self, "classifier_cls_%d" % c) for c in range(Cf)]
        w0 = torch.stack([b[0].weight for b in blocks], 0)
        main = w0[:, :, :C].reshape(Cf * 128, C, 3, 3)
        extra = w0[:, :, C]
        eye = torch.eye(Cf, device=w0.device, dtype=w0.dtype)
        blk = (extra[:, :, None] * eye[:, None, :, None, None]).reshape(Cf * 128, Cf, 3, 3)
        w1 = torch.cat([main, blk], 1)
        b1 = torch.cat([b[0].bias for b in blocks], 0)
        w2s = torch.stack([b[2].weight[0] for b in blocks], 0)
        w2 = (w2s[:, None] * eye[:, :, None, None, None]).reshape(Cf, Cf * 128, 3, 3)
        b2 = torch.cat([b[2].bias for b in blocks], 0)
        return w1, b1, w2, b2

    def _logits(self, feature, act_maps, shape, grl_applied=False):
        Cf = self.num_classes
        if not grl_applied:
            feature = self.grad_reverse(feature)
            act_maps = self.grad_reverse(act_maps)
        cs1 = ops.pad4(self.in_channels + Cf)
        if ops.CAT_IN_PLACE and self.num_convs > 0:
            buf = feature.new_empty((feature.shape[0], cs1))
            x = run_tower(self.dis_tower, feature, shape, self.num_convs, out_buf=buf)
            xcat = ops.cat_into(x, act_maps[:, 1:], buf)
        else:
            x = run_tower(self.dis_tower, feature, shape, self.num_convs)
            xcat = torch.cat([x, act_maps[:, 1:]], 1)
            if cs1 != xcat.shape[1]:
                xcat = torch.nn.functional.pad(xcat, (0, cs1 - xcat.shape[1]))
        blocks = [getattr(self, "classifier_cls_%d" % c) for c in range(Cf)]
        if ops.BATCHED and Cf <= ops.CKA_STACK_MAX:
            w1, b1, w2, b2 = ops.cka_stacked_weights([(b[0], b[2]) for b in blocks], self.in_channels, 128,
                                                     xcat.shape[1])
        else:
            w1, b1, w2, b2 = self._stacked_weights_torch()
        h = ops.conv2d(xcat, w1, b1, shape, 3, 1, relu="deferred")
        if ops.GROUPED_CLS and 1 <= Cf <= ops.gconv_max_groups():
            if not w2.permute(0, 2, 3, 1).is_contiguous():
                w2 = w2.contiguous(memory_format=torch.channels_last)
            return ops.gconv3x3_to1(h, w2, b2, shape, Cf, mask_dx=True)[:, :Cf], act_maps
        return ops.conv2d(h, w2, b2, shape, 3, 1, mask_dx=True)[:, :Cf], act_maps

    def _loss(self, logits, act_maps, target):
        Cf = self.num_classes
        if Cf == 1:
            logits = logits.reshape(-1)
            return ops.bce_with_logits_mean(logits, torch.full_like(logits, float(target)))
        return ops.cka_bce(logits, act_maps.detach(), float(target), Cf)

    def forward(self, feature, target, act_maps=None, domain="source", shape=None):
        assert target in (0, 1, 0.1, 0.9) and domain in ("source", "target")
        logits, act_maps = self._logits(feature, act_maps, shape)
        return self._loss(logits, act_maps, target)

    def forward_pair(self, feature, act_maps, shape, n_src, grl_applied=False):
        logits, act_maps = self._logits(feature, act_maps, shape, grl_applied)
        (h, w) = shape.sizes[0]
        m = n_src * h * w
        if self.num_classes > 1 and 0 < m < logits.shape[0]:
            return ops.cka_bce_pair(logits, act_maps.detach(), m, self.num_classes)
        ls, lt = ops.split_rows2(logits, m)
        return self._loss(ls, act_maps[:m], 1.0), self._loss(lt, act_maps[m:], 0.0)
```

scan_amd/ops.py:

```python
import contextlib
import ctypes
import os
import weakref

import torch

from . import _lib
from ._lib import PyramidDesc, call, query


def _ptr(t):
    return ctypes.c_void_p(t.data_ptr()) if t is not None else ctypes.c_void_p(0)


def _stream():
    return ctypes.c_void_p(torch._C._cuda_getCurrentRawStream(torch._C._cuda_getDevice()))


def _chk(*ts):
    for t in ts:
        if t is None:
            continue
        if not t.is_cuda:
            raise RuntimeError("scan_amd ops run only on the GPU (HIP) -- got a %s tensor; no CPU fallback" % t.device)
# ... 1293 lines not shown
        logits, act, out_s, out_t = ctx.saved_tensors
        m, cf = ctx.cfg
        M = logits.shape[0]
        d = torch.empty_like(logits)
        for lo, hi, target, g, out in ((0, m, 1.0, gs, out_s), (m, M, 0.0, gt, out_t)):
            if g is None:
                d[lo:hi].zero_()
            else:
                call("scan_cka_bce_backward_loss", _ptr(logits[lo:hi]), _ptr(act[lo:hi]), hi - lo, cf, target,
                     _ptr(g.reshape(1).contiguous()), _ptr(out), _ptr(d[lo:hi]), _stream())
        return d, None, None, None


def cka_bce_pair(logits, act_detached, m, cf):
    return _CkaBcePair.apply(logits.contiguous(), act_detached.contiguous(), int(m), int(cf))


class _SplitRows2(torch.autograd.Function):

    @staticmethod
    def forward(ctx, x, m):
        ctx.m = m
        ctx.shape = x.shape
        return x[:m], x[m:]

    @staticmethod
    def backward(ctx, g1, g2):
        m = ctx.m
        g = (g1 if g1 is not None else g2).new_empty(ctx.shape)
        if g1 is not None:
            g[:m] = g1
        else:
            g[:m].zero_()
        if g2 is not None:
            g[m:] = g2
        else:
            g[m:].zero_()
        return g, None


def split_rows2(x, m):
    return _SplitRows2.apply(x, m)


def cka_bce(logits, act_detached, target, cf):
    return _CkaBce.apply(logits.contiguous(), act_detached.contiguous(), float(target), int(cf))


class _SoftmaxFocalMean(torch.autograd.Function):
    @staticmethod
    def forward(ctx, logits, labels, gamma):
        _chk(logits, labels)
        if labels.dtype != torch.int64:
            raise RuntimeError("labels must be int64")
        M, K = logits.shape
        out = logits.new_zeros((1,))
        _call_reduction("scan_softmax_focal", "_forward", logits, (M,), _ptr(logits), _ptr(labels), M, K, gamma, _ptr(out))
        ctx.save_for_backward(logits, labels)
        ctx.gamma = gamma
        return out[0] / M

    @staticmethod
    def backward(ctx, g):
        logits, labels = ctx.saved_tensors
        M, K = logits.shape
        d = torch.empty_like(logits)
        call("scan_softmax_focal_backward", _ptr(logits), _ptr(labels), M, K, ctx.gamma, 1.0 / M, _ptr(d), _stream())
        return d * g, None, None


def softmax_focal_loss_mean(logits, labels, gamma=2.0):
    return _SoftmaxFocalMean.apply(logits.contiguous(), labels.contiguous(), float(gamma))


class _GradReverse(torch.autograd.Function):

    @staticmethod
    def forward(ctx, x, lam):
        if not x.is_cuda:
            raise RuntimeError("scan_amd ops run only on the GPU (HIP) -- got a %s tensor; no CPU fallback" % x.device)
        ctx.lam = lam
        return x.view_as(x)

    @staticmethod
    def backward(ctx, g):
        if not (g.is_contiguous() or (g.dim() == 4 and g.is_contiguous(memory_format=torch.channels_last))):
            g = g.contiguous()
        d = torch.empty_like(g)
        call("scan_scale", _ptr(g), -ctx.lam, _ptr(d), g.numel(), _stream())
        return d, None


def grad_reverse(x, lam):
    return _GradReverse.apply(x, float(lam))


def _nms_impl(dets, scores, labels, thr, rule_ge):
    n = dets.shape[0]
    if n == 0:
        return torch.empty((0,), dtype=torch.int64, device="cpu")
    _chk(dets, scores, labels)
    if n > _lib.NMS_MAX:
        raise RuntimeError("nms: n=%d exceeds SCAN_NMS_MAX=%d" % (n, _lib.NMS_MAX))
    dets = dets.contiguous().float()
    scores = scores.contiguous().float()
    if labels is not None:
        labels = labels.contiguous().float()
    keep, cnt = _nms_launch(dets, scores, labels, thr, rule_ge)
    return keep[:int(cnt.item())]


def _nms_launch(dets, scores, labels, thr, rule_ge):
    n = dets.shape[0]
    ws = torch.empty((query("scan_nms_ws_bytes", n) + 15) // 16 * 2, dtype=torch.float64, device=dets.device)
    keep = torch.empty((n,), dtype=torch.int64, device=dets.device)
    cnt = torch.empty((1,), dtype=torch.int32, device=dets.device)
    call("scan_nms", _ptr(dets), _ptr(scores), _ptr(labels), n, float(thr), int(rule_ge), _ptr(keep), _ptr(cnt),
         _ptr(ws), _stream())
    return keep, cnt


def nms_by_label_async(dets, scores, labels, thr):
    n = dets.shape[0]
    if n == 0:
        return lambda: torch.empty((0,), dtype=torch.int64, device="cpu")
    _chk(dets, scores, labels)
    if n > _lib.NMS_MAX:
        raise RuntimeError("nms: n=%d exceeds SCAN_NMS_MAX=%d" % (n, _lib.NMS_MAX))
    keep, cnt = _nms_launch(dets.contiguous().float(), scores.contiguous().float(), labels.contiguous().float(), thr, True)
    return lambda: keep[:int(cnt.item())]


def nms(dets, scores, thr, rule_ge=True):
    return _nms_impl(dets, scores, None, thr, rule_ge)


def nms_by_label(dets, scores, labels, thr):
    return _nms_impl(dets, scores, labels.float(), thr, True)


def ml_nms(dets, scores, labels, thr):
    return _nms_impl(dets, scores, labels, thr, False)


def dbscan_in_cluster0(pts, eps, min_samples=5):
    _chk(pts)
    n, d = pts.shape
    if n == 0:
        return torch.zeros((0,), dtype=torch.bool, device=pts.device)
    nbytes = query("scan_dbscan_ws_bytes", n)
    if nbytes < 0:
        raise RuntimeError("dbscan: n=%d exceeds SCAN_DBSCAN_MAX" % n)
    ws = torch.empty((nbytes // 8 + 1,), dtype=torch.float64, device=pts.device)
    info = torch.empty((2,), dtype=torch.int32, device=pts.device)
    st = _stream()
    call("scan_dbscan_prepare", _ptr(pts), n, d, float(eps), int(min_samples), _ptr(ws), _ptr(info), st)
    if int(info[0].item()) >= n:
        return torch.zeros((n,), dtype=torch.bool, device=pts.device)
    changed = torch.zeros((1,), dtype=torch.int32, device=pts.device)
    parity = 0
    while True:
        call("scan_dbscan_bfs_step", n, _ptr(ws), parity, _ptr(changed), st)
        if int(changed.item()) == 0:
            break
        parity ^= 1
    out = torch.empty((n,), dtype=torch.uint8, device=pts.device)
    call("scan_dbscan_finish", n, _ptr(ws), _ptr(out), st)
    return out.bool()


class _CkaStackedWeights(torch.autograd.Function):

    @staticmethod
    def forward(ctx, C, H, cs1, *params):
        cf = len(params) // 4
        w0s, b0s, w2s, b2s = params[0::4], params[1::4], params[2::4], params[3::4]
        for t in params:
            if not t.is_cuda or t.dtype != torch.float32:
                raise RuntimeError("scan_amd ops run only on fp32 GPU (HIP) tensors -- got %s %s; no CPU fallback"
                                   % (t.device, t.dtype))
        w0, w2 = w0s[0], w2s[0]
        assert tuple(w0.shape) == (H, C + 1, 3, 3) and tuple(w2.shape) == (1, H, 3, 3), (w0.shape, w2.shape)
        for a, b in zip(w0s, w2s):
            if a.stride() != w0.stride() or b.stride() != w2.stride() or a.shape != w0.shape or b.shape != w2.shape:
                raise RuntimeError("cka_stacked_weights: the class branches must share one memory layout")
        if w0.stride(2) != 3 * w0.stride(3) or w2.stride(2) != 3 * w2.stride(3):
            raise RuntimeError("cka_stacked_weights: the 3x3 taps of a weight must be evenly strided")
        strides = (w0.stride(0), w0.stride(1), w0.stride(3), w2.stride(1), w2.stride(3))
        cs2 = cf * H
        dev = w0.device
        w1 = torch.empty((cf * H, 9, cs1), device=dev)
        b1 = torch.empty((cf * H,), device=dev)
        w2o = torch.empty((cf, 9, cs2), device=dev)
        b2 = torch.empty((cf,), device=dev)
        arr = (_lib.CkaBranch * cf)()
        for a, p0, q0, p2, q2 in zip(arr, w0s, b0s, w2s, b2s):
            a.w0, a.b0, a.w2, a.b2 = p0.data_ptr(), q0.data_ptr(), p2.data_ptr(), q2.data_ptr()
        call("scan_cka_stack_weights", arr, cf, C, H, *strides, cs1, cs2, _ptr(w1), _ptr(b1), _ptr(w2o), _ptr(b2),
             _stream())
        ctx.cfg = (cf, C, H, cs1, cs2, strides)
        ctx.params = params
        return (w1.view(cf * H, 3, 3, cs1).permute(0, 3, 1, 2), b1, w2o.view(cf, 3, 3, cs2).permute(0, 3, 1, 2), b2)

    @staticmethod
    def backward(ctx, dw1, db1, dw2, db2):
        cf, C, H, cs1, cs2, strides = ctx.cfg
        params = ctx.params

        def ohwi(g):
            return None if g is None else g.permute(0, 2, 3, 1).contiguous()

        dw1, dw2 = ohwi(dw1), ohwi(dw2)
        db1 = None if db1 is None else db1.contiguous()
        db2 = None if db2 is None else db2.contiguous()
        direct = all(getattr(p, "_scan_flat", False) and p.grad is not None and p.grad.stride() == p.stride()
                     for p in params)
        tgt = [p.grad for p in params] if direct else [torch.zeros_like(p) for p in params]
        arr = (_lib.CkaBranch * cf)()
        for c, a in enumerate(arr):
            a.w0, a.b0, a.w2, a.b2 = (t.data_ptr() for t in tgt[4 * c:4 * c + 4])
        call("scan_cka_unstack_grads", arr, cf, C, H, *strides, cs1, cs2, _ptr(dw1), _ptr(db1), _ptr(dw2), _ptr(db2),
             1, _stream())
        return (None, None, None) + (tuple(None for _ in params) if direct else tuple(tgt))


CKA_STACK_MAX = _lib.CKA_MAX_CLASSES


def cka_stacked_weights(branches, C, H, cs1):
    params = []
    for c0, c2 in branches:
        params += [c0.weight, c0.bias, c2.weight, c2.bias]
    return _CkaStackedWeights.apply(int(C), int(H), int(cs1), *params)


class _GroupedConvTo1(torch.autograd.Function):

    @staticmethod
    def forward(ctx, x, w, bias, shape, G, mask_dx):
        _chk(x, bias)
        gc = G * 128
        assert x.shape == (shape.rows, gc) and tuple(w.shape) == (G, gc, 3, 3) and w.permute(0, 2, 3, 1).is_contiguous()
        ns = pad4(G)
        y = x.new_empty((shape.rows, ns))
        ws = x.new_empty((query("scan_gconv3x3_to1_ws_floats", shape.ref(), G, 128),))
        bits = None
        mfma = query("scan_tune_get", b"gconv_mfma")
        any_ = "" if G in (1, 2, 4, 8) else "any_"
        if mfma == 1 and not any_ and mask_dx and torch.is_grad_enabled() and x.requires_grad:
            bits = torch.empty((shape.rows * G * 4,), dtype=torch.int32, device=x.device)
            call("scan_gconv3x3_to1_forward_bits", _ptr(x), shape.ref(), G, 128, _ptr(w), _ptr(bias), _ptr(y), ns,
                 _ptr(ws), _ptr(bits), _stream())
        else:
            call("scan_gconv3x3_to1_%sforward" % any_, _ptr(x), shape.ref(), G, 128, _ptr(w), _ptr(bias), _ptr(y), ns, _ptr(ws),
                 _stream())
        ctx.save_for_backward(x, w, bits)
        ctx.cfg = (shape, G, ns, mask_dx, bias is not None)
        return y

    @staticmethod
    def backward(ctx, dy):
        x, w, bits = ctx.saved_tensors
        shape, G, ns, mask_dx, has_bias = ctx.cfg
        any_ = "" if G in (1, 2, 4, 8) else "any_"
        dy = dy.contiguous()
        st = _stream()
        dx = dw = db = dwp = None
        if ctx.needs_input_grad[1]:
            dwp = x.new_zeros((G, 9, G * 128))
            ws = x.new_empty((query("scan_gconv3x3_to1_ws_floats", shape.ref(), G, 128),))
            dw = dwp.view(G, 3, 3, G * 128).permute(0, 3, 1, 2)
        if ctx.needs_input_grad[0]:
            dx = torch.empty_like(x)
        if dx is not None and dwp is not None and bits is not None:
            call("scan_gconv3x3_to1_backward_bits", _ptr(x), _ptr(dy), ns, shape.ref(), G, 128, _ptr(w), _ptr(bits),
                 _ptr(dx), _ptr(dwp), 0, _ptr(ws), st)
        elif dx is not None and dwp is not None:
            call("scan_gconv3x3_to1_%sbackward" % any_, _ptr(x), _ptr(dy), ns, shape.ref(), G, 128, _ptr(w), int(mask_dx), _ptr(dx),
                 _ptr(dwp), 0, _ptr(ws), st)
        elif dx is not None:
            call("scan_gconv3x3_to1_%sdgrad" % any_, _ptr(dy), ns, shape.ref(), G, 128, _ptr(w), _ptr(x if mask_dx else None),
                 _ptr(dx), st)
        elif dwp is not None:
            call("scan_gconv3x3_to1_%swgrad" % any_, _ptr(x), _ptr(dy), ns, shape.ref(), G, 128, _ptr(dwp), 0, _ptr(ws), st)
        if has_bias and ctx.needs_input_grad[2]:
            M = dy.shape[0]
            cws = x.new_empty((query("scan_colsum_ws_floats", M, G),))
            db = x.new_empty((G,))
            call("scan_colsum", _ptr(dy), M, G, ns, _ptr(db), 0, _ptr(cws), st)
        return dx, dw, db, None, None, None


GROUPED_CLS = os.environ.get("SCAN_GROUPED_CLS", "1") != "0"


def gconv_max_groups():
    return _limit("scan_gconv3x3_to1_max_groups")


def gconv3x3_to1(x, w, bias, shape, G, mask_dx=False):
    return _GroupedConvTo1.apply(x, w, bias, shape, int(G), bool(mask_dx))


COND_RNN_FUSED = os.environ.get("SCAN_COND_RNN", "1") != "0"


class _CondRnn(torch.autograd.Function):

    @staticmethod
    def forward(ctx, proto, *params):
        if not (proto.is_cuda and all(p.is_cuda and p.dtype == torch.float32 for p in params)):
            raise RuntimeError("scan_amd ops run only on the GPU (HIP); no CPU fallback")
        K, C, T = proto.shape
        proto = proto.permute(2, 0, 1).contiguous()
        ws_ = [p.detach().contiguous() for p in params]
        h0 = proto.new_empty((T, K, 512))
        h1 = torch.empty_like(h0)
        ker = proto.new_empty((K, 256))
        wptr = (ctypes.c_void_p * 10)(*[w.data_ptr() for w in ws_])
        call("scan_cond_rnn_forward", _ptr(proto), K, T, wptr, _ptr(h0), _ptr(h1), _ptr(ker), _stream())
        ctx.save_for_backward(proto, h0, h1, *ws_)
        return ker

    @staticmethod
    def backward(ctx, dker):
        proto, h0, h1, *ws_ = ctx.saved_tensors
        T, K, C = proto.shape
        dker = dker.contiguous()
        grads = [torch.empty_like(w) for w in ws_]
        wptr = (ctypes.c_void_p * 10)(*[w.data_ptr() for w in ws_])
        gptr = (ctypes.c_void_p * 10)(*[g.data_ptr() for g in grads])
        ws = proto.new_empty((query("scan_cond_rnn_ws_floats"),))
        call("scan_cond_rnn_backward", _ptr(proto), K, T, wptr, _ptr(h0), _ptr(h1), _ptr(dker), gptr, _ptr(ws), _stream())
        return (None, *grads)


def cond_rnn_supported(proto, params):
    K, C, T = proto.shape
    return (COND_RNN_FUSED and proto.is_cuda and K <= 9 and T <= 3 and C == 256 and tuple(params[0].shape) == (512, 256)
            and tuple(params[8].shape[:3]) == (256, 512, T))


def cond_rnn(proto, params):
    return _CondRnn.apply(proto, *params)


def sgd_momentum_multi_(segments, momentum):
    segments = [sg for sg in segments if sg[0].numel() > 0]
    for k in range(0, len(segments), _lib.SGD_MAX_SEGMENTS):
        part = segments[k:k + _lib.SGD_MAX_SEGMENTS]
        arr = (_lib.SgdSegment * len(part))()
        for a, (p, g, buf, lr, wd, first) in zip(arr, part):
            _chk(p, g, buf)
            assert p.numel() == g.numel() == buf.numel()
            a.p, a.g, a.buf, a.n = p.data_ptr(), g.data_ptr(), buf.data_ptr(), p.numel()
            a.lr, a.wd, a.first_step, a.reserved = float(lr), float(wd), int(bool(first)), 0
        call("scan_sgd_momentum_multi", arr, len(part), float(momentum), _stream())


def sgd_momentum_(p, g, buf, lr, wd, momentum, first_step):
    _chk(p, g, buf)
    call("scan_sgd_momentum", _ptr(p), _ptr(g), _ptr(buf), p.numel(), float(lr), float(wd), float(momentum),
         int(first_step), _stream())
```

Before: 25.04.

## Split CKA activation-map channel out of first classifier conv into fused grouped kernel

The per-class classifier's first 3x3 conv used to take a concatenated input (tower features plus one activation-map channel per class), which required building a padded concat buffer. Now the main conv runs only on the tower output with shared weights. Each class's activation-map tap contribution, together with the bias-free ReLU, is folded into a new grouped to-1 conv kernel that adds a*E to the hidden units on the fly. The backward pass is fused as well, with new stack and unstack kernels for the split weights. This removes the concat and the extra input channels from the large conv, at the cost of recomputing the hidden activation inside the grouped kernel and adding a lot of new code.

New measurement: 25.55, median of 6. 1.02x the previous value.

```diff
diff --git a/include/scan_hip.h b/include/scan_hip.h
--- a/include/scan_hip.h
+++ b/include/scan_hip.h
@@ -373,6 +373,12 @@
 int scan_cka_unstack_grads(const scan_cka_branch_t* grads, int32_t Cf, int32_t C, int32_t H, int64_t s1o, int64_t s1c,
                            int64_t s1k, int64_t s2c, int64_t s2k, int32_t Cs1, int32_t Cs2, const float* dw1,
                            const float* db1, const float* dw2, const float* db2, int32_t accumulate, void* stream);
+int scan_cka_stack_weights_split(const scan_cka_branch_t* branches, int32_t Cf, int32_t C, int32_t H, int64_t s1o, int64_t s1c,
+                                 int64_t s1k, int64_t s2c, int64_t s2k, int32_t Cs2, float* wmain, float* e, float* b1,
+                                 float* w2, float* b2, void* stream);
+int scan_cka_unstack_grads_split(const scan_cka_branch_t* grads, int32_t Cf, int32_t C, int32_t H, int64_t s1o, int64_t s1c,
+                                 int64_t s1k, int64_t s2c, int64_t s2k, int32_t Cs2, const float* dwmain, const float* de,
+                                 const float* db1, const float* dw2, const float* db2, int32_t accumulate, void* stream);
 
 int64_t scan_gconv3x3_to1_ws_floats(const scan_pyramid_t* d, int32_t G, int32_t Cg);
 int scan_gconv3x3_to1_forward(const float* x, const scan_pyramid_t* d, int32_t G, int32_t Cg, const float* w,
@@ -394,6 +400,20 @@
 int scan_gconv3x3_to1_any_backward(const float* x, const float* dy, int32_t Ns, const scan_pyramid_t* d, int32_t G, int32_t Cg,
                                    const float* w, int32_t relu_mask, float* dx, float* dw, int32_t accumulate, float* ws,
                                    void* stream);
+int64_t scan_gconv3x3_to1_act_ws_floats(const scan_pyramid_t* d, int32_t G, int32_t Cg);
+int scan_gconv3x3_to1_act_forward(const float* x, const scan_pyramid_t* d, int32_t G, int32_t Cg, const float* w,
+                                  const float* bias, const float* a, int32_t lda, int32_t a_col0, const float* E, float* y,
+                                  int32_t Ns, float* ws, void* stream);
+int scan_gconv3x3_to1_act_backward(const float* x, const float* dy, int32_t Ns, const scan_pyramid_t* d, int32_t G, int32_t Cg,
+                                   const float* w, const float* a, int32_t lda, int32_t a_col0, const float* E, float* dx,
+                                   float* dw, int32_t accumulate, float* ws, void* stream);
+int scan_gconv3x3_to1_act_grads(const float* dh, const scan_pyramid_t* d, int32_t G, int32_t Cg, const float* a, int32_t lda,
+                                int32_t a_col0, const float* E, float* da, int32_t ldda, int32_t da_col0, float* dE,
+                                int32_t accumulate, float* ws, void* stream);
+int scan_gconv3x3_to1_act_backward_all(const float* x, const float* dy, int32_t Ns, const scan_pyramid_t* d, int32_t G,
+                                       int32_t Cg, const float* w, const float* a, int32_t lda, int32_t a_col0, const float* E,
+                                       float* dx, float* dw, float* da, int32_t ldda, int32_t da_col0, float* dE,
+                                       int32_t accumulate, float* ws, void* stream);
 int scan_gconv3x3_to1_forward_bits(const float* x, const scan_pyramid_t* d, int32_t G, int32_t Cg, const float* w,
                                    const float* bias, float* y, int32_t Ns, float* ws, uint32_t* relu_bits, void* stream);
 int scan_gconv3x3_to1_backward_bits(const float* x, const float* dy, int32_t Ns, const scan_pyramid_t* d, int32_t G,
diff --git a/scan_amd/_lib.py b/scan_amd/_lib.py
--- a/scan_amd/_lib.py
+++ b/scan_amd/_lib.py
@@ -208,6 +208,19 @@
     "scan_gconv3x3_to1_forward_bits": (ctypes.c_int, [c_vp, _PD, c_i32, c_i32, c_vp, c_vp, c_vp, c_i32, c_vp, c_vp, c_vp]),
     "scan_gconv3x3_to1_backward_bits": (ctypes.c_int, [c_vp, c_vp, c_i32, _PD, c_i32, c_i32, c_vp, c_vp, c_vp, c_vp, c_i32,
                                                        c_vp, c_vp]),
+    "scan_cka_stack_weights_split": (ctypes.c_int, [ctypes.POINTER(CkaBranch), c_i32, c_i32, c_i32, c_i64, c_i64, c_i64, c_i64,
+                                                    c_i64, c_i32, c_vp, c_vp, c_vp, c_vp, c_vp, c_vp]),
+    "scan_cka_unstack_grads_split": (ctypes.c_int, [ctypes.POINTER(CkaBranch), c_i32, c_i32, c_i32, c_i64, c_i64, c_i64, c_i64,
+                                                    c_i64, c_i32, c_vp, c_vp, c_vp, c_vp, c_vp, c_i32, c_vp]),
+    "scan_gconv3x3_to1_act_ws_floats": (c_i64, [_PD, c_i32, c_i32]),
+    "scan_gconv3x3_to1_act_forward": (ctypes.c_int, [c_vp, _PD, c_i32, c_i32, c_vp, c_vp, c_vp, c_i32, c_i32, c_vp, c_vp, c_i32,
+                                                     c_vp, c_vp]),
+    "scan_gconv3x3_to1_act_backward": (ctypes.c_int, [c_vp, c_vp, c_i32, _PD, c_i32, c_i32, c_vp, c_vp, c_i32, c_i32, c_vp, c_vp,
+                                                      c_vp, c_i32, c_vp, c_vp]),
+    "scan_gconv3x3_to1_act_backward_all": (ctypes.c_int, [c_vp, c_vp, c_i32, _PD, c_i32, c_i32, c_vp, c_vp, c_i32, c_i32, c_vp,
+                                                          c_vp, c_vp, c_vp, c_i32, c_i32, c_vp, c_i32, c_vp, c_vp]),
+    "scan_gconv3x3_to1_act_grads": (ctypes.c_int, [c_vp, _PD, c_i32, c_i32, c_vp, c_i32, c_i32, c_vp, c_vp, c_i32, c_i32, c_vp,
+                                                   c_i32, c_vp, c_vp]),
     "scan_resize_bilinear_u8": (ctypes.c_int, [c_vp, c_i32, c_i32, c_vp, c_vp, c_i32, c_i32, c_vp, c_vp, c_i32, c_vp, c_vp,
                                                c_i32, c_vp]),
     "scan_sigmoid_focal_loss_ordered_ws_floats": (c_i64, [c_i64, c_i32]),
diff --git a/scan_amd/csrc/batched.hip b/scan_amd/csrc/batched.hip
--- a/scan_amd/csrc/batched.hip
+++ b/scan_amd/csrc/batched.hip
@@ -204,11 +204,13 @@
 __global__ __launch_bounds__(256) void cka_stack_kernel(CkaPtrs P, int Cf, int C, int H, int64_t s1o, int64_t s1c,
                                                         int64_t s1k, int64_t s2c, int64_t s2k, int Cs1, int Cs2,
                                                         float* __restrict__ w1, float* __restrict__ b1,
-                                                        float* __restrict__ w2, float* __restrict__ b2) {
+                                                        float* __restrict__ w2, float* __restrict__ b2,
+                                                        float* __restrict__ e) {
   const int64_t n1 = (int64_t)Cf * H * 9 * Cs1;
   const int64_t n2 = (int64_t)Cf * 9 * Cs2;
   const int64_t nb = (int64_t)Cf * H + Cf;
-  for (int64_t i = (int64_t)blockIdx.x * blockDim.x + threadIdx.x; i < n1 + n2 + nb;
+  const int64_t ne = e != nullptr ? (int64_t)Cf * 9 * H : 0;
+  for (int64_t i = (int64_t)blockIdx.x * blockDim.x + threadIdx.x; i < n1 + n2 + nb + ne;
        i += (int64_t)gridDim.x * blockDim.x) {
     if (i < n1) {
       const int col = (int)(i % Cs1);
@@ -218,7 +220,7 @@
       const int c = row / H, o = row - c * H;
       float v = 0.f;
       if (col < C) v = P.b[c].w0[o * s1o + col * s1c + k * s1k];
-      else if (col == C + c) v = P.b[c].w0[o * s1o + C * s1c + k * s1k];
+      else if (e == nullptr && col == C + c) v = P.b[c].w0[o * s1o + C * s1c + k * s1k];
       w1[i] = v;
     } else if (i < n1 + n2) {
       const int64_t q = i - n1;
@@ -229,10 +231,17 @@
       float v = 0.f;
       if (col >= c * H && col < (c + 1) * H) v = P.b[c].w2[(col - c * H) * s2c + k * s2k];
       w2[q] = v;
-    } else {
+    } else if (i < n1 + n2 + nb) {
       const int q = (int)(i - n1 - n2);
       if (q < Cf * H) b1[q] = P.b[q / H].b0[q % H];
       else b2[q - Cf * H] = P.b[q - Cf * H].b2[0];
+    } else {
+      const int64_t q = i - n1 - n2 - nb;
+      const int o = (int)(q % H);
+      const int64_t r = q / H;
+      const int k = (int)(r % 9);
+      const int c = (int)(r / 9);
+      e[q] = P.b[c].w0[o * s1o + C * s1c + k * s1k];
     }
   }
 }
@@ -241,7 +250,7 @@
                                                           int64_t s1k, int64_t s2c, int64_t s2k, int Cs1, int Cs2,
                                                           const float* __restrict__ dw1, const float* __restrict__ db1,
                                                           const float* __restrict__ dw2, const float* __restrict__ db2,
-                                                          int accumulate) {
+                                                          const float* __restrict__ de, int accumulate) {
   const int64_t n1 = (int64_t)Cf * H * 9 * (C + 1);
   const int64_t n2 = (int64_t)Cf * 9 * H;
   const int64_t nb = (int64_t)Cf * H + Cf;
@@ -253,7 +262,13 @@
       const int k = (int)(r % 9);
       const int row = (int)(r / 9);
       const int c = row / H, o = row - c * H;
-      if (dw1 != nullptr) {
+      if (Cs1 == C && col == C) {
+        if (de != nullptr) {
+          float* dst = const_cast<float*>(G.b[c].w0) + o * s1o + col * s1c + k * s1k;
+          const float v = de[((int64_t)c * 9 + k) * H + o];
+          *dst = accumulate ? *dst + v : v;
+        }
+      } else if (dw1 != nullptr) {
         const float v = dw1[((int64_t)row * 9 + k) * Cs1 + (col < C ? col : C + c)];
         float* dst = const_cast<float*>(G.b[c].w0) + o * s1o + col * s1c + k * s1k;
         *dst = accumulate ? *dst + v : v;
@@ -284,9 +299,11 @@
   }
 }
 
-static int cka_check(const scan_cka_branch_t* br, int Cf, int C, int H, int Cs1, int Cs2, const char* who) {
+static int cka_check(const scan_cka_branch_t* br, int Cf, int C, int H, int Cs1, int Cs2, const char* who,
+                     bool split = false) {
   SCAN_CHECK_ARG(br && Cf >= 1 && Cf <= SCAN_CKA_MAX_CLASSES, "%s: Cf=%d out of 1..%d", who, Cf, SCAN_CKA_MAX_CLASSES);
-  SCAN_CHECK_ARG(C > 0 && H > 0 && Cs1 >= C + Cf && Cs2 >= Cf * H, "%s: C=%d H=%d Cs1=%d Cs2=%d", who, C, H, Cs1, Cs2);
+  SCAN_CHECK_ARG(C > 0 && H > 0 && Cs1 >= C + (split ? 0 : Cf) && Cs2 >= Cf * H, "%s: C=%d H=%d Cs1=%d Cs2=%d", who, C, H,
+                 Cs1, Cs2);
   for (int c = 0; c < Cf; ++c)
     SCAN_CHECK_ARG(br[c].w0 && br[c].b0 && br[c].w2 && br[c].b2, "%s: null pointer in branch %d", who, c);
   return 0;
@@ -301,8 +318,22 @@
   for (int c = 0; c < Cf; ++c) P.b[c] = branches[c];
   const int64_t n = (int64_t)Cf * H * 9 * Cs1 + (int64_t)Cf * 9 * Cs2 + (int64_t)Cf * H + Cf;
   hipLaunchKernelGGL(cka_stack_kernel, dim3(grid_for(n, 256)), dim3(256), 0, as_stream(stream), P, Cf, C, H, s1o, s1c,
-                     s1k, s2c, s2k, Cs1, Cs2, w1, b1, w2, b2);
+                     s1k, s2c, s2k, Cs1, Cs2, w1, b1, w2, b2, (float*)nullptr);
   SCAN_LAUNCH_CHECK("cka_stack_weights");
+  return 0;
+}
+
+extern "C" int scan_cka_stack_weights_split(const scan_cka_branch_t* branches, int32_t Cf, int32_t C, int32_t H, int64_t s1o,
+                                            int64_t s1c, int64_t s1k, int64_t s2c, int64_t s2k, int32_t Cs2, float* wmain,
+                                            float* e, float* b1, float* w2, float* b2, void* stream) {
+  if (cka_check(branches, Cf, C, H, C, Cs2, "cka_stack_weights_split", true)) return -1;
+  SCAN_CHECK_ARG(wmain && e && b1 && w2 && b2, "cka_stack_weights_split: null output");
+  CkaPtrs P;
+  for (int c = 0; c < Cf; ++c) P.b[c] = branches[c];
+  const int64_t n = (int64_t)Cf * H * 9 * C + (int64_t)Cf * 9 * Cs2 + (int64_t)Cf * H + Cf + (int64_t)Cf * 9 * H;
+  hipLaunchKernelGGL(cka_stack_kernel, dim3(grid_for(n, 256)), dim3(256), 0, as_stream(stream), P, Cf, C, H, s1o, s1c,
+                     s1k, s2c, s2k, C, Cs2, wmain, b1, w2, b2, e);
+  SCAN_LAUNCH_CHECK("cka_stack_weights_split");
   return 0;
 }
 
@@ -315,7 +346,21 @@
   for (int c = 0; c < Cf; ++c) G.b[c] = grads[c];
   const int64_t n = (int64_t)Cf * H * 9 * (C + 1) + (int64_t)Cf * 9 * H + (int64_t)Cf * H + Cf;
   hipLaunchKernelGGL(cka_unstack_kernel, dim3(grid_for(n, 256)), dim3(256), 0, as_stream(stream), G, Cf, C, H, s1o, s1c,
-                     s1k, s2c, s2k, Cs1, Cs2, dw1, db1, dw2, db2, accumulate);
+                     s1k, s2c, s2k, Cs1, Cs2, dw1, db1, dw2, db2, (const float*)nullptr, accumulate);
   SCAN_LAUNCH_CHECK("cka_unstack_grads");
   return 0;
 }
+
+extern "C" int scan_cka_unstack_grads_split(const scan_cka_branch_t* grads, int32_t Cf, int32_t C, int32_t H, int64_t s1o,
+                                            int64_t s1c, int64_t s1k, int64_t s2c, int64_t s2k, int32_t Cs2,
+                                            const float* dwmain, const float* de, const float* db1, const float* dw2,
+                                            const float* db2, int32_t accumulate, void* stream) {
+  if (cka_check(grads, Cf, C, H, C, Cs2, "cka_unstack_grads_split", true)) return -1;
+  CkaPtrs G;
+  for (int c = 0; c < Cf; ++c) G.b[c] = grads[c];
+  const int64_t n = (int64_t)Cf * H * 9 * (C + 1) + (int64_t)Cf * 9 * H + (int64_t)Cf * H + Cf;
+  hipLaunchKernelGGL(cka_unstack_kernel, dim3(grid_for(n, 256)), dim3(256), 0, as_stream(stream), G, Cf, C, H, s1o, s1c,
+                     s1k, s2c, s2k, C, Cs2, dwmain, db1, dw2, db2, de, accumulate);
+  SCAN_LAUNCH_CHECK("cka_unstack_grads_split");
+  return 0;
+}
diff --git a/scan_amd/csrc/gconv.hip b/scan_amd/csrc/gconv.hip
--- a/scan_amd/csrc/gconv.hip
+++ b/scan_amd/csrc/gconv.hip
@@ -648,3 +648,397 @@
   return gconv_backward(x, dy, Ns, d, G, Cg, w, relu_mask, nullptr, dx, dw, accumulate, ws, as_stream(stream),
                         "gconv3x3_to1_any_backward", true);
 }
+
+
+template <int SIGN>
+__device__ __forceinline__ void tap_values(const scan_pyramid_t& d, int64_t q, const RowCoord& rc,
+                                           const float* __restrict__ src, int ld, int g, bool uniform, float (&v)[9]) {
+  if (uniform) {
+    const int g0 = 2 * (int)(threadIdx.x >> 6);
+    const int l = threadIdx.x & 63;
+    const int tl = l % 9, gl = l / 9;
+    const int64_t pl = l < 18 ? neighbour_row(d, q, rc, SIGN * (tl / 3 - 1), SIGN * (tl % 3 - 1)) : -1;
+    const float val = pl >= 0 ? src[pl * ld + g0 + gl] : 0.f;
+    const int vb = __builtin_bit_cast(int, val);
+    const bool hi = (l & 32) != 0;
+#pragma unroll
+    for (int t = 0; t < 9; ++t) {
+      const float lo_v = __builtin_bit_cast(float, __builtin_amdgcn_readlane(vb, t));
+      const float hi_v = __builtin_bit_cast(float, __builtin_amdgcn_readlane(vb, 9 + t));
+      v[t] = hi ? hi_v : lo_v;
+    }
+  } else {
+#pragma unroll
+    for (int t = 0; t < 9; ++t) {
+      const int64_t p = neighbour_row(d, q, rc, SIGN * (t / 3 - 1), SIGN * (t % 3 - 1));
+      v[t] = p >= 0 ? src[p * ld + g] : 0.f;
+    }
+  }
+}
+
+__device__ __forceinline__ float4 act_hidden(float4 h, const float4 (&ev)[9], const float (&av)[9]) {
+#pragma unroll
+  for (int t = 0; t < 9; ++t) {
+    h.x = __fmaf_rn(av[t], ev[t].x, h.x);
+    h.y = __fmaf_rn(av[t], ev[t].y, h.y);
+    h.z = __fmaf_rn(av[t], ev[t].z, h.z);
+    h.w = __fmaf_rn(av[t], ev[t].w, h.w);
+  }
+  h.x = h.x > 0.f ? h.x : 0.f;
+  h.y = h.y > 0.f ? h.y : 0.f;
+  h.z = h.z > 0.f ? h.z : 0.f;
+  h.w = h.w > 0.f ? h.w : 0.f;
+  return h;
+}
+
+__device__ __forceinline__ int64_t uniform_row(int64_t q) {
+  return ((int64_t)__builtin_amdgcn_readfirstlane((int)(q >> 32)) << 32) | (uint32_t)__builtin_amdgcn_readfirstlane((int)q);
+}
+
+#define GC_UNROLL_A 2
+
+template <bool UNI>
+__global__ __launch_bounds__(256) void gconv_taps_act_kernel(const float* __restrict__ x, scan_pyramid_t d, int G, int GC,
+                                                             const float* __restrict__ w, const float* __restrict__ a,
+                                                             int lda, const float* __restrict__ E, float* __restrict__ T) {
+  const int64_t M = d.row_off[d.n_levels];
+  const int quads = GC >> 2, slots = 256 / quads;
+  const int cq = threadIdx.x % quads, slot = threadIdx.x / quads;
+  const int g = cq >> 5, l32 = cq & 31;
+  float4 wv[9], ev[9];
+#pragma unroll
+  for (int t = 0; t < 9; ++t) {
+    wv[t] = *reinterpret_cast<const float4*>(w + ((int64_t)g * 9 + t) * GC + 4 * cq);
+    ev[t] = *reinterpret_cast<const float4*>(E + ((int64_t)g * 9 + t) * GC_G + 4 * l32);
+  }
+  const int64_t stride = (int64_t)gridDim.x * slots;
+  for (int64_t q0 = (int64_t)blockIdx.x * slots + slot; q0 < M; q0 += GC_UNROLL_F * stride) {
+    float4 h[GC_UNROLL_F];
+#pragma unroll
+    for (int u = 0; u < GC_UNROLL_F; ++u) {
+      const int64_t q = q0 + u * stride;
+      h[u] = q < M ? *reinterpret_cast<const float4*>(x + q * GC + 4 * cq) : make_float4(0.f, 0.f, 0.f, 0.f);
+    }
+#pragma unroll
+    for (int u = 0; u < GC_UNROLL_F; ++u) {
+      int64_t q = q0 + u * stride;
+      if (UNI) q = uniform_row(q);
+      if (q >= M) continue;
+      float av[9];
+      tap_values<1>(d, q, decode_row(d, q), a, lda, g, UNI, av);
+      const float4 hv = act_hidden(h[u], ev, av);
+      float mine = 0.f;
+#pragma unroll
+      for (int t = 0; t < 9; ++t) {
+        float s = __fmaf_rn(hv.x, wv[t].x, __fmaf_rn(hv.y, wv[t].y, __fmaf_rn(hv.z, wv[t].z, hv.w * wv[t].w)));
+        s = half_wave_sum_hi(s);
+        if (l32 == 16 + t) mine = s;
+      }
+      if (l32 >= 16 && l32 < 25) T[(q * G + g) * 9 + (l32 - 16)] = mine;
+    }
+  }
+}
+
+__device__ __forceinline__ void slab_store(const float4 (&acc)[9], float* __restrict__ red, float* __restrict__ slab, int GC,
+                                           int quads, int slots, int cq, int slot) {
+  float* out = slab + (int64_t)blockIdx.x * 9 * GC;
+  if (slots == 1) {
+#pragma unroll
+    for (int t = 0; t < 9; ++t) *reinterpret_cast<float4*>(out + (int64_t)t * GC + 4 * cq) = acc[t];
+    return;
+  }
+#pragma unroll
+  for (int t = 0; t < 9; ++t) *reinterpret_cast<float4*>(red + (t * 256 + threadIdx.x) * 4) = acc[t];
+  __syncthreads();
+  if (slot == 0) {
+#pragma unroll
+    for (int t = 0; t < 9; ++t) {
+      float4 s = acc[t];
+      for (int k = 1; k < slots; ++k) {
+        const float4 v = *reinterpret_cast<const float4*>(red + (t * 256 + k * quads + cq) * 4);
+        s.x += v.x;
+        s.y += v.y;
+        s.z += v.z;
+        s.w += v.w;
+      }
+      *reinterpret_cast<float4*>(out + (int64_t)t * GC + 4 * cq) = s;
+    }
+  }
+}
+
+template <bool UNI, bool FUSE>
+__global__ __launch_bounds__(256, (UNI && !FUSE) ? 3 : 2) void gconv_bwd_act_kernel(
+    const float* __restrict__ x, const float* __restrict__ dy, int Ns, scan_pyramid_t d, int G, int GC,
+    const float* __restrict__ w, const float* __restrict__ a, int lda, const float* __restrict__ E, float* __restrict__ dx,
+    float* __restrict__ slab, float* __restrict__ T, float* __restrict__ slab_e) {
+  __shared__ float red[9 * 1024];
+  const int64_t M = d.row_off[d.n_levels];
+  const int quads = GC >> 2, slots = 256 / quads;
+  const int cq = threadIdx.x % quads, slot = threadIdx.x / quads;
+  const int g = cq >> 5, l32 = cq & 31;
+  float4 wv[9], ev[9], acc[9], acc_e[9];
+#pragma unroll
+  for (int t = 0; t < 9; ++t) {
+    wv[t] = *reinterpret_cast<const float4*>(w + ((int64_t)g * 9 + t) * GC + 4 * cq);
+    ev[t] = *reinterpret_cast<const float4*>(E + ((int64_t)g * 9 + t) * GC_G + 4 * l32);
+    acc[t] = make_float4(0.f, 0.f, 0.f, 0.f);
+    if (FUSE) acc_e[t] = make_float4(0.f, 0.f, 0.f, 0.f);
+  }
+  for (int64_t q0 = (int64_t)blockIdx.x * GC_UNROLL_A * slots + slot; q0 < M;
+       q0 += (int64_t)gridDim.x * GC_UNROLL_A * slots) {
+    float4 h[GC_UNROLL_A];
+#pragma unroll
+    for (int u = 0; u < GC_UNROLL_A; ++u) {
+      const int64_t q = q0 + u * slots;
+      h[u] = q < M ? *reinterpret_cast<const float4*>(x + q * GC + 4 * cq) : make_float4(0.f, 0.f, 0.f, 0.f);
+    }
+#pragma unroll
+    for (int u = 0; u < GC_UNROLL_A; ++u) {
+      int64_t q = q0 + u * slots;
+      if (UNI) q = uniform_row(q);
+      if (q >= M) continue;
+      const RowCoord rc = decode_row(d, q);
+      float av[9], gy[9];
+      tap_values<1>(d, q, rc, a, lda, g, UNI, av);
+      const float4 hv = act_hidden(h[u], ev, av);
+      tap_values<-1>(d, q, rc, dy, Ns, g, UNI, gy);
+      float4 o = make_float4(0.f, 0.f, 0.f, 0.f);
+#pragma unroll
+      for (int t = 0; t < 9; ++t) {
+        acc[t].x = __fmaf_rn(gy[t], hv.x, acc[t].x);
+        acc[t].y = __fmaf_rn(gy[t], hv.y, acc[t].y);
+        acc[t].z = __fmaf_rn(gy[t], hv.z, acc[t].z);
+        acc[t].w = __fmaf_rn(gy[t], hv.w, acc[t].w);
+        o.x = __fmaf_rn(gy[t], wv[t].x, o.x);
+        o.y = __fmaf_rn(gy[t], wv[t].y, o.y);
+        o.z = __fmaf_rn(gy[t], wv[t].z, o.z);
+        o.w = __fmaf_rn(gy[t], wv[t].w, o.w);
+      }
+      o.x = hv.x > 0.f ? o.x : 0.f;
+      o.y = hv.y > 0.f ? o.y : 0.f;
+      o.z = hv.z > 0.f ? o.z : 0.f;
+      o.w = hv.w > 0.f ? o.w : 0.f;
+      *reinterpret_cast<float4*>(dx + q * GC + 4 * cq) = o;
+      if (FUSE) {
+        float mine = 0.f;
+#pragma unroll
+        for (int t = 0; t < 9; ++t) {
+          acc_e[t].x = __fmaf_rn(av[t], o.x, acc_e[t].x);
+          acc_e[t].y = __fmaf_rn(av[t], o.y, acc_e[t].y);
+          acc_e[t].z = __fmaf_rn(av[t], o.z, acc_e[t].z);
+          acc_e[t].w = __fmaf_rn(av[t], o.w, acc_e[t].w);
+          float s = __fmaf_rn(o.x, ev[8 - t].x, __fmaf_rn(o.y, ev[8 - t].y, __fmaf_rn(o.z, ev[8 - t].z, o.w * ev[8 - t].w)));
+          s = half_wave_sum_hi(s);
+          if (l32 == 16 + t) mine = s;
+        }
+        if (l32 >= 16 && l32 < 25) T[(q * G + g) * 9 + (l32 - 16)] = mine;
+      }
+    }
+  }
+  slab_store(acc, red, slab, GC, quads, slots, cq, slot);
+  if (FUSE) {
+    __syncthreads();
+    slab_store(acc_e, red, slab_e, GC, quads, slots, cq, slot);
+  }
+}
+
+template <bool UNI>
+__global__ __launch_bounds__(256) void gconv_act_grads_kernel(const float* __restrict__ dh, scan_pyramid_t d, int G, int GC,
+                                                              const float* __restrict__ a, int lda,
+                                                              const float* __restrict__ E, float* __restrict__ T,
+                                                              float* __restrict__ slab) {
+  __shared__ float red[9 * 1024];
+  const int64_t M = d.row_off[d.n_levels];
+  const int quads = GC >> 2, slots = 256 / quads;
+  const int cq = threadIdx.x % quads, slot = threadIdx.x / quads;
+  const int g = cq >> 5, l32 = cq & 31;
+  float4 ev[9], acc[9];
+#pragma unroll
+  for (int t = 0; t < 9; ++t) {
+    ev[t] = *reinterpret_cast<const float4*>(E + ((int64_t)g * 9 + t) * GC_G + 4 * l32);
+    acc[t] = make_float4(0.f, 0.f, 0.f, 0.f);
+  }
+  for (int64_t q0 = (int64_t)blockIdx.x * GC_UNROLL_A * slots + slot; q0 < M;
+       q0 += (int64_t)gridDim.x * GC_UNROLL_A * slots) {
+    float4 h[GC_UNROLL_A];
+#pragma unroll
+    for (int u = 0; u < GC_UNROLL_A; ++u) {
+      const int64_t q = q0 + u * slots;
+      h[u] = q < M ? *reinterpret_cast<const float4*>(dh + q * GC + 4 * cq) : make_float4(0.f, 0.f, 0.f, 0.f);
+    }
+#pragma unroll
+    for (int u = 0; u < GC_UNROLL_A; ++u) {
+      int64_t q = q0 + u * slots;
+      if (UNI) q = uniform_row(q);
+      if (q >= M) continue;
+      float av[9];
+      tap_values<1>(d, q, decode_row(d, q), a, lda, g, UNI, av);
+      float mine = 0.f;
+#pragma unroll
+      for (int t = 0; t < 9; ++t) {
+        acc[t].x = __fmaf_rn(av[t], h[u].x, acc[t].x);
+        acc[t].y = __fmaf_rn(av[t], h[u].y, acc[t].y);
+        acc[t].z = __fmaf_rn(av[t], h[u].z, acc[t].z);
+        acc[t].w = __fmaf_rn(av[t], h[u].w, acc[t].w);
+        float s = __fmaf_rn(h[u].x, ev[8 - t].x,
+                            __fmaf_rn(h[u].y, ev[8 - t].y, __fmaf_rn(h[u].z, ev[8 - t].z, h[u].w * ev[8 - t].w)));
+        s = half_wave_sum_hi(s);
+        if (l32 == 16 + t) mine = s;
+      }
+      if (l32 >= 16 && l32 < 25) T[(q * G + g) * 9 + (l32 - 16)] = mine;
+    }
+  }
+  slab_store(acc, red, slab, GC, quads, slots, cq, slot);
+}
+
+__global__ __launch_bounds__(256) void gconv_gather_cols_kernel(const float* __restrict__ T, scan_pyramid_t d, int G,
+                                                                float* __restrict__ y, int ldy, int col0) {
+  const int64_t M = d.row_off[d.n_levels];
+  for (int64_t i = (int64_t)blockIdx.x * blockDim.x + threadIdx.x; i < M * ldy; i += (int64_t)gridDim.x * blockDim.x) {
+    const int64_t p = i / ldy;
+    const int g = (int)(i - p * ldy) - col0;
+    float acc = 0.f;
+    if (g >= 0 && g < G) {
+      const RowCoord rc = decode_row(d, p);
+#pragma unroll
+      for (int t = 0; t < 9; ++t) {
+        const int64_t q = neighbour_row(d, p, rc, t / 3 - 1, t % 3 - 1);
+        if (q >= 0) acc += T[(q * G + g) * 9 + t];
+      }
+    }
+    y[i] = acc;
+  }
+}
+
+__global__ __launch_bounds__(256) void gconv_act_reduce_kernel(const float* __restrict__ partial, int parts, int GC,
+                                                               float* __restrict__ dE, int accumulate) {
+  const int i = blockIdx.x * blockDim.x + threadIdx.x;
+  if (i >= 9 * GC) return;
+  const int t = i / GC, c = i - t * GC;
+  float s = 0.f;
+  for (int b = 0; b < parts; ++b) s += partial[(int64_t)b * 9 * GC + i];
+  float* dst = dE + ((int64_t)(c / GC_G) * 9 + t) * GC_G + c % GC_G;
+  *dst = accumulate ? *dst + s : s;
+}
+
+static int gconv_act_check(const scan_pyramid_t* d, int G, int Cg, const float* a, int lda, int a_col0, const float* E,
+                           const char* who) {
+  if (gconv_check(d, G, Cg, who)) return -1;
+  SCAN_CHECK_ARG(a && E && a_col0 >= 0 && lda >= a_col0 + G, "%s: bad act map (lda=%d, first column %d, G=%d)", who, lda,
+                 a_col0, G);
+  return 0;
+}
+
+static int gconv_slab_blocks(int64_t M) {
+  int64_t rpb = (M + GC_MAX_BLOCKS - 1) / GC_MAX_BLOCKS;
+  if (rpb < 16) rpb = 16;
+  return (int)((M + rpb - 1) / rpb);
+}
+
+static int gconv_slab_reduce(float* slab, int blocks, int GC, float** partial, hipStream_t st) {
+  const int n = 9 * GC, per = (blocks + GC_PARTS - 1) / GC_PARTS, parts = (blocks + per - 1) / per;
+  *partial = slab + (int64_t)GC_MAX_BLOCKS * n;
+  hipLaunchKernelGGL(gconv_slab_partial_kernel, dim3((n + 255) / 256, parts), dim3(256), 0, st, slab, blocks, n, per,
+                     *partial);
+  return parts;
+}
+
+extern "C" int64_t scan_gconv3x3_to1_act_ws_floats(const scan_pyramid_t* d, int32_t G, int32_t Cg) {
+  if (!d) return -1;
+  const int64_t M = d->row_off[d->n_levels];
+  return M * G * 9 + 2 * (int64_t)(GC_MAX_BLOCKS + GC_PARTS) * 9 * G * Cg;
+}
+
+extern "C" int scan_gconv3x3_to1_act_forward(const float* x, const scan_pyramid_t* d, int32_t G, int32_t Cg, const float* w,
+                                             const float* bias, const float* a, int32_t lda, int32_t a_col0, const float* E,
+                                             float* y, int32_t Ns, float* ws, void* stream) {
+  if (gconv_act_check(d, G, Cg, a, lda, a_col0, E, "gconv3x3_to1_act_forward")) return -1;
+  SCAN_CHECK_ARG(x && w && y && ws && Ns >= G, "gconv3x3_to1_act_forward: bad arguments (Ns=%d)", Ns);
+  const int64_t M = d->row_off[d->n_levels];
+  if (M == 0) return 0;
+  const int GC = G * Cg, slots = 256 / (GC / 4);
+  hipStream_t st = as_stream(stream);
+  hipLaunchKernelGGL((G == 8 ? gconv_taps_act_kernel<true> : gconv_taps_act_kernel<false>), dim3(grid_for((M + slots - 1) / slots, 1)), dim3(256), 0, st, x, *d, G, GC, w,
+                     a + a_col0, lda, E, ws);
+  SCAN_LAUNCH_CHECK("gconv_taps_act");
+  hipLaunchKernelGGL(gconv_gather_kernel, dim3(grid_for(M * Ns, 256)), dim3(256), 0, st, ws, *d, G, bias, y, Ns);
+  SCAN_LAUNCH_CHECK("gconv_gather");
+  return 0;
+}
+
+extern "C" int scan_gconv3x3_to1_act_backward(const float* x, const float* dy, int32_t Ns, const scan_pyramid_t* d, int32_t G,
+                                              int32_t Cg, const float* w, const float* a, int32_t lda, int32_t a_col0,
+                                              const float* E, float* dx, float* dw, int32_t accumulate, float* ws,
+                                              void* stream) {
+  if (gconv_act_check(d, G, Cg, a, lda, a_col0, E, "gconv3x3_to1_act_backward")) return -1;
+  SCAN_CHECK_ARG(x && dy && w && dx && dw && ws && Ns >= G, "gconv3x3_to1_act_backward: bad arguments (Ns=%d)", Ns);
+  const int64_t M = d->row_off[d->n_levels];
+  if (M == 0) return 0;
+  const int GC = G * Cg, blocks = gconv_slab_blocks(M);
+  hipStream_t st = as_stream(stream);
+  hipLaunchKernelGGL((G == 8 ? gconv_bwd_act_kernel<true, false> : gconv_bwd_act_kernel<false, false>), dim3(blocks), dim3(256),
+                     0, st, x, dy, Ns, *d, G, GC, w, a + a_col0, lda, E, dx, ws, (float*)nullptr, (float*)nullptr);
+  SCAN_LAUNCH_CHECK("gconv_bwd_act");
+  float* partial;
+  const int parts = gconv_slab_reduce(ws, blocks, GC, &partial, st);
+  SCAN_LAUNCH_CHECK("gconv_slab_partial");
+  hipLaunchKernelGGL(gconv_wgrad_reduce_kernel, dim3((9 * GC + 255) / 256), dim3(256), 0, st, partial, parts, G, GC, dw,
+                     accumulate);
+  SCAN_LAUNCH_CHECK("gconv_wgrad_reduce");
+  return 0;
+}
+
+extern "C" int scan_gconv3x3_to1_act_grads(const float* dh, const scan_pyramid_t* d, int32_t G, int32_t Cg, const float* a,
+                                           int32_t lda, int32_t a_col0, const float* E, float* da, int32_t ldda,
+                                           int32_t da_col0, float* dE, int32_t accumulate, float* ws, void* stream) {
+  if (gconv_act_check(d, G, Cg, a, lda, a_col0, E, "gconv3x3_to1_act_grads")) return -1;
+  SCAN_CHECK_ARG(dh && da && dE && ws && da_col0 >= 0 && ldda >= da_col0 + G,
+                 "gconv3x3_to1_act_grads: bad arguments (ldda=%d, first column %d)", ldda, da_col0);
+  const int64_t M = d->row_off[d->n_levels];
+  if (M == 0) return 0;
+  const int GC = G * Cg, blocks = gconv_slab_blocks(M);
+  hipStream_t st = as_stream(stream);
+  float* slab = ws + M * G * 9;
+  hipLaunchKernelGGL((G == 8 ? gconv_act_grads_kernel<true> : gconv_act_grads_kernel<false>), dim3(blocks), dim3(256), 0, st, dh, *d, G, GC, a + a_col0, lda, E, ws, slab);
+  SCAN_LAUNCH_CHECK("gconv_act_grads");
+  hipLaunchKernelGGL(gconv_gather_cols_kernel, dim3(grid_for(M * ldda, 256)), dim3(256), 0, st, ws, *d, G, da, ldda, da_col0);
+  SCAN_LAUNCH_CHECK("gconv_gather_cols");
+  float* partial;
+  const int parts = gconv_slab_reduce(slab, blocks, GC, &partial, st);
+  SCAN_LAUNCH_CHECK("gconv_slab_partial");
+  hipLaunchKernelGGL(gconv_act_reduce_kernel, dim3((9 * GC + 255) / 256), dim3(256), 0, st, partial, parts, GC, dE, accumulate);
+  SCAN_LAUNCH_CHECK("gconv_act_reduce");
+  return 0;
+}
+
+extern "C" int scan_gconv3x3_to1_act_backward_all(const float* x, const float* dy, int32_t Ns, const scan_pyramid_t* d,
+                                                  int32_t G, int32_t Cg, const float* w, const float* a, int32_t lda,
+                                                  int32_t a_col0, const float* E, float* dx, float* dw, float* da, int32_t ldda,
+                                                  int32_t da_col0, float* dE, int32_t accumulate, float* ws, void* stream) {
+  if (gconv_act_check(d, G, Cg, a, lda, a_col0, E, "gconv3x3_to1_act_backward_all")) return -1;
+  SCAN_CHECK_ARG(x && dy && w && dx && dw && ws && Ns >= G, "gconv3x3_to1_act_backward_all: bad arguments (Ns=%d)", Ns);
+  SCAN_CHECK_ARG(da && dE && da_col0 >= 0 && ldda >= da_col0 + G,
+                 "gconv3x3_to1_act_backward_all: bad arguments (ldda=%d, first column %d)", ldda, da_col0);
+  const int64_t M = d->row_off[d->n_levels];
+  if (M == 0) return 0;
+  const int GC = G * Cg, blocks = gconv_slab_blocks(M);
+  hipStream_t st = as_stream(stream);
+  float* slab = ws + M * G * 9;
+  float* slab_e = slab + (int64_t)(GC_MAX_BLOCKS + GC_PARTS) * 9 * GC;
+  hipLaunchKernelGGL((G == 8 ? gconv_bwd_act_kernel<true, true> : gconv_bwd_act_kernel<false, true>), dim3(blocks), dim3(256), 0,
+                     st, x, dy, Ns, *d, G, GC, w, a + a_col0, lda, E, dx, slab, ws, slab_e);
+  SCAN_LAUNCH_CHECK("gconv_bwd_act");
+  hipLaunchKernelGGL(gconv_gather_cols_kernel, dim3(grid_for(M * ldda, 256)), dim3(256), 0, st, ws, *d, G, da, ldda, da_col0);
+  SCAN_LAUNCH_CHECK("gconv_gather_cols");
+  float* partial;
+  int parts = gconv_slab_reduce(slab, blocks, GC, &partial, st);
+  SCAN_LAUNCH_CHECK("gconv_slab_partial");
+  hipLaunchKernelGGL(gconv_wgrad_reduce_kernel, dim3((9 * GC + 255) / 256), dim3(256), 0, st, partial, parts, G, GC, dw,
+                     accumulate);
+  SCAN_LAUNCH_CHECK("gconv_wgrad_reduce");
+  parts = gconv_slab_reduce(slab_e, blocks, GC, &partial, st);
+  SCAN_LAUNCH_CHECK("gconv_slab_partial");
+  hipLaunchKernelGGL(gconv_act_reduce_kernel, dim3((9 * GC + 255) / 256), dim3(256), 0, st, partial, parts, GC, dE, accumulate);
+  SCAN_LAUNCH_CHECK("gconv_act_reduce");
+  return 0;
+}
diff --git a/scan_amd/modeling/discriminator.py b/scan_amd/modeling/discriminator.py
--- a/scan_amd/modeling/discriminator.py
+++ b/scan_amd/modeling/discriminator.py
@@ -128,6 +128,12 @@
         if not grl_applied:
             feature = self.grad_reverse(feature)
             act_maps = self.grad_reverse(act_maps)
+        blocks = [getattr(self, "classifier_cls_%d" % c) for c in range(Cf)]
+        if ops.CLS_SPLIT and ops.BATCHED and ops.GROUPED_CLS and ops.cls_split_supported(Cf):
+            x = run_tower(self.dis_tower, feature, shape, self.num_convs)
+            wm, e, b1, w2, b2 = ops.cka_stacked_weights_split([(b[0], b[2]) for b in blocks], self.in_channels, 128)
+            h = ops.conv2d(x, wm, b1, shape, 3, 1)
+            return ops.gconv3x3_to1_act(h, w2, b2, act_maps, e, shape, Cf, 1)[:, :Cf], act_maps
         cs1 = ops.pad4(self.in_channels + Cf)
         if ops.CAT_IN_PLACE and self.num_convs > 0:
             buf = feature.new_empty((feature.shape[0], cs1))
@@ -138,7 +144,6 @@
             xcat = torch.cat([x, act_maps[:, 1:]], 1)
             if cs1 != xcat.shape[1]:
                 xcat = torch.nn.functional.pad(xcat, (0, cs1 - xcat.shape[1]))
-        blocks = [getattr(self, "classifier_cls_%d" % c) for c in range(Cf)]
         if ops.BATCHED and Cf <= ops.CKA_STACK_MAX:
             w1, b1, w2, b2 = ops.cka_stacked_weights([(b[0], b[2]) for b in blocks], self.in_channels, 128,
                                                      xcat.shape[1])
diff --git a/scan_amd/ops.py b/scan_amd/ops.py
--- a/scan_amd/ops.py
+++ b/scan_amd/ops.py
@@ -1619,6 +1619,140 @@
     return _GroupedConvTo1.apply(x, w, bias, shape, int(G), bool(mask_dx))
 
 
+CLS_SPLIT = os.environ.get("SCAN_CLS_SPLIT", "1") != "0"
+
+
+CLS_SPLIT_FUSED = os.environ.get("SCAN_CLS_SPLIT_FUSED", "1") != "0"
+
+
+def cls_split_supported(G):
+    return G in (1, 2, 4, 8) and query("scan_tune_get", b"gconv_mfma") == 0
+
+
+class _CkaStackedWeightsSplit(torch.autograd.Function):
+
+    @staticmethod
+    def forward(ctx, C, H, *params):
+        cf = len(params) // 4
+        w0s, b0s, w2s, b2s = params[0::4], params[1::4], params[2::4], params[3::4]
+        for t in params:
+            if not t.is_cuda or t.dtype != torch.float32:
+                raise RuntimeError("scan_amd ops run only on fp32 GPU (HIP) tensors -- got %s %s; no CPU fallback"
+                                   % (t.device, t.dtype))
+        w0, w2 = w0s[0], w2s[0]
+        assert tuple(w0.shape) == (H, C + 1, 3, 3) and tuple(w2.shape) == (1, H, 3, 3), (w0.shape, w2.shape)
+        for a, b in zip(w0s, w2s):
+            if a.stride() != w0.stride() or b.stride() != w2.stride() or a.shape != w0.shape or b.shape != w2.shape:
+                raise RuntimeError("cka_stacked_weights_split: the class branches must share one memory layout")
+        if w0.stride(2) != 3 * w0.stride(3) or w2.stride(2) != 3 * w2.stride(3):
+            raise RuntimeError("cka_stacked_weights_split: the 3x3 taps of a weight must be evenly strided")
+        strides = (w0.stride(0), w0.stride(1), w0.stride(3), w2.stride(1), w2.stride(3))
+        cs2 = cf * H
+        dev = w0.device
+        wm = torch.empty((cf * H, 9, C), device=dev)
+        e = torch.empty((cf, 9, H), device=dev)
+        b1 = torch.empty((cf * H,), device=dev)
+        w2o = torch.empty((cf, 9, cs2), device=dev)
+        b2 = torch.empty((cf,), device=dev)
+        arr = (_lib.CkaBranch * cf)()
+        for a, p0, q0, p2, q2 in zip(arr, w0s, b0s, w2s, b2s):
+            a.w0, a.b0, a.w2, a.b2 = p0.data_ptr(), q0.data_ptr(), p2.data_ptr(), q2.data_ptr()
+        call("scan_cka_stack_weights_split", arr, cf, C, H, *strides, cs2, _ptr(wm), _ptr(e), _ptr(b1), _ptr(w2o), _ptr(b2),
+             _stream())
+        ctx.cfg = (cf, C, H, cs2, strides)
+        ctx.params = params
+        return (wm.view(cf * H, 3, 3, C).permute(0, 3, 1, 2), e, b1, w2o.view(cf, 3, 3, cs2).permute(0, 3, 1, 2), b2)
+
+    @staticmethod
+    def backward(ctx, dwm, de, db1, dw2, db2):
+        cf, C, H, cs2, strides = ctx.cfg
+        params = ctx.params
+
+        def ohwi(g):
+            return None if g is None else g.permute(0, 2, 3, 1).contiguous()
+
+        dwm, dw2 = ohwi(dwm), ohwi(dw2)
+        de, db1, db2 = (None if g is None else g.contiguous() for g in (de, db1, db2))
+        direct = all(getattr(p, "_scan_flat", False) and p.grad is not None and p.grad.stride() == p.stride()
+                     for p in params)
+        tgt = [p.grad for p in params] if direct else [torch.zeros_like(p) for p in params]
+        arr = (_lib.CkaBranch * cf)()
+        for c, a in enumerate(arr):
+            a.w0, a.b0, a.w2, a.b2 = (t.data_ptr() for t in tgt[4 * c:4 * c + 4])
+        call("scan_cka_unstack_grads_split", arr, cf, C, H, *strides, cs2, _ptr(dwm), _ptr(de), _ptr(db1), _ptr(dw2),
+             _ptr(db2), 1, _stream())
+        return (None, None) + (tuple(None for _ in params) if direct else tuple(tgt))
+
+
+def cka_stacked_weights_split(branches, C, H):
+    params = []
+    for c0, c2 in branches:
+        params += [c0.weight, c0.bias, c2.weight, c2.bias]
+    return _CkaStackedWeightsSplit.apply(int(C), int(H), *params)
+
+
+class _GroupedConvTo1Act(torch.autograd.Function):
+
+    @staticmethod
+    def forward(ctx, h, w, bias, act, e, shape, G, col0):
+        _chk(h, bias, act, e)
+        gc = G * 128
+        assert h.shape == (shape.rows, gc) and tuple(w.shape) == (G, gc, 3, 3) and w.permute(0, 2, 3, 1).is_contiguous()
+        assert act.shape[0] == shape.rows and act.shape[1] >= col0 + G and act.is_contiguous(), (act.shape, col0, G)
+        assert tuple(e.shape) == (G, 9, 128) and e.is_contiguous() and h.is_contiguous()
+        if not cls_split_supported(G):
+            raise RuntimeError("gconv3x3_to1_act: G=%d on the fp32 FMA kernels only (G in 1, 2, 4, 8; gconv_mfma = 0)" % G)
+        ns = pad4(G)
+        y = h.new_empty((shape.rows, ns))
+        ws = h.new_empty((query("scan_gconv3x3_to1_act_ws_floats", shape.ref(), G, 128),))
+        call("scan_gconv3x3_to1_act_forward", _ptr(h), shape.ref(), G, 128, _ptr(w), _ptr(bias), _ptr(act), act.shape[1], col0,
+             _ptr(e), _ptr(y), ns, _ptr(ws), _stream())
+        ctx.save_for_backward(h, w, act, e)
+        ctx.cfg = (shape, G, ns, col0, bias is not None)
+        return y
+
+    @staticmethod
+    def backward(ctx, dy):
+        h, w, act, e = ctx.saved_tensors
+        shape, G, ns, col0, has_bias = ctx.cfg
+        dy = dy.contiguous()
+        st = _stream()
+        K = act.shape[1]
+        ws = h.new_empty((query("scan_gconv3x3_to1_act_ws_floats", shape.ref(), G, 128),))
+        dwp = h.new_zeros((G, 9, G * 128))
+        dh = torch.empty_like(h)
+        want_act = ctx.needs_input_grad[3] or ctx.needs_input_grad[4]
+        fused = CLS_SPLIT_FUSED and want_act
+        if fused:
+            dact, de = torch.empty_like(act), torch.empty_like(e)
+            call("scan_gconv3x3_to1_act_backward_all", _ptr(h), _ptr(dy), ns, shape.ref(), G, 128, _ptr(w), _ptr(act), K, col0,
+                 _ptr(e), _ptr(dh), _ptr(dwp), _ptr(dact), K, col0, _ptr(de), 0, _ptr(ws), st)
+        else:
+            call("scan_gconv3x3_to1_act_backward", _ptr(h), _ptr(dy), ns, shape.ref(), G, 128, _ptr(w), _ptr(act), K, col0,
+                 _ptr(e), _ptr(dh), _ptr(dwp), 0, _ptr(ws), st)
+        dw = dwp.view(G, 3, 3, G * 128).permute(0, 3, 1, 2) if ctx.needs_input_grad[1] else None
+        db = None
+        if not fused:
+            dact = de = None
+        if has_bias and ctx.needs_input_grad[2]:
+            M = dy.shape[0]
+            cws = h.new_empty((query("scan_colsum_ws_floats", M, G),))
+            db = h.new_empty((G,))
+            call("scan_colsum", _ptr(dy), M, G, ns, _ptr(db), 0, _ptr(cws), st)
+        if want_act and not fused:
+            dact = torch.empty_like(act)
+            de = torch.empty_like(e)
+            call("scan_gconv3x3_to1_act_grads", _ptr(dh), shape.ref(), G, 128, _ptr(act), K, col0, _ptr(e), _ptr(dact), K, col0,
+                 _ptr(de), 0, _ptr(ws), st)
+        dact = dact if ctx.needs_input_grad[3] else None
+        de = de if ctx.needs_input_grad[4] else None
+        return (dh if ctx.needs_input_grad[0] else None), dw, db, dact, de, None, None, None
+
+
+def gconv3x3_to1_act(h, w, bias, act, e, shape, G, col0=1):
+    return _GroupedConvTo1Act.apply(h, w, bias, act.contiguous(), e, shape, int(G), int(col0))
+
+
 COND_RNN_FUSED = os.environ.get("SCAN_COND_RNN", "1") != "0"
 
 
```
